# HTDerekLiu/surface_multigrid_code

Hardware: AMD Instinct MI355X
Metric: V-cycles/sec + fine-level SpMV GB/s (% HBM peak), 1M-vert mesh fp64 (higher is better)
Workload: dtype f64; 1 GPU; C3: bunny_15K_init x3 midpoint subdivision, 1011330 verts, 5 levels, M_bary+0.01(-L), fp64; n_verts=1011330, nnz=7079298, levels=5, smoother=gs, rhs_columns_per_gpu=1, parallelism=single GPU

## Files before the change

### surface_multigrid_code_amd/csrc/smg_capi.cpp

```cpp
#include <hip/hip_runtime.h>

#include <algorithm>
#include <atomic>
#include <chrono>
#include <cmath>
#include <cstdarg>
#include <cstdio>
#include <cstdlib>
#include <cstring>
#include <functional>
#include <memory>
#include <numeric>
#include <string>
#include <thread>
#include <vector>

#include "smg_internal.hpp"

using namespace smg;

static thread_local std::string g_err;
int smg::fail(int code, const char* fmt, ...)
{
    char buf[512];
    va_list ap;
    va_start(ap, fmt);
    std::vsnprintf(buf, sizeof(buf), fmt, ap);
    va_end(ap);
    g_err = buf;
    return code;
}

extern "C" const char* smg_last_error(void) { return g_err.c_str(); }
extern "C" int smg_version(void) { return SMG_VERSION; }
extern "C" long long smg_device_bytes_live(void) { return (long long)smg::devbuf_live_bytes().load(); }
extern "C" int smg_debug_device_bytes(const smg_hierarchy* h, char* buf, int cap)
{
    if (!h || !buf || cap < 1) return SMG_ERR_INVALID;
    std::string out;
    auto B = [](const auto& d) { return (long long)(d.n * sizeof(*d.p)); };
    auto sell = [&](const smg::SellBuf& S) { return B(S.slice_row) + B(S.slice_off) + B(S.slice_w) + B(S.col) + B(S.order) + B(S.val) + B(S.diag_slot) + B(S.long_row) + B(S.long_ptr) + B(S.long_col) + B(S.long_val) + B(S.long_valf); };
    long long tot = 0;
    auto line = [&](const std::string& nm, long long v) { if (v) { out += nm + " " + std::to_string(v) + "\n"; tot += v; } };
    for (int lv = 0; lv < h->n_levels; lv++) {
        const smg::Level& L = h->lv[lv];
        const std::string p = "level" + std::to_string(lv) + ".";
        line(p + "A_sell", sell(L.dA)); line(p + "AT_sell", sell(L.dAT)); line(p + "P_sell", sell(L.dP)); line(p + "PT_sell", sell(L.dPT));
        line(p + "A_block3", B(L.bA.slice_row) + B(L.bA.slice_off) + B(L.bA.slice_w) + B(L.bA.col) + B(L.bA.order) + B(L.bA.val) + B(L.bA.valf) + B(L.bAT.slice_row) + B(L.bAT.slice_off) + B(L.bAT.slice_w) + B(L.bAT.col) + B(L.bAT.order) + B(L.bAT.val) + B(L.bAT.valf) + B(L.mapB) + B(L.mapBT));
        line(p + "values_caller_order", B(L.d_Aval) + B(L.d_Tval));
        line(p + "refresh_maps", B(L.mapA) + B(L.mapAT));
        line(p + "galerkin_recipes", B(L.r1_ptr) + B(L.r1_idx) + B(L.r2_ptr) + B(L.r2_idx) + B(L.r1_coef) + B(L.r2_coef));
        long long t = 0;
        for (const auto& T : L.tiled) t += B(T.hdr) + B(T.ext_rows) + B(T.pcol) + B(T.prow) + B(T.map) + B(T.mapd) + B(T.pval) + B(T.pdiag);
        line(p + "tiled_plans", t);
        line(p + "bgs_plan", B(L.bgs.hdr) + B(L.bgs.xrow) + B(L.bgs.ugrow) + B(L.bgs.ulrow) + B(L.bgs.eidx) + B(L.bgs.map) + B(L.bgs.mapd) + B(L.bgs.eval) + B(L.bgs.udiag));
        line(p + "wgs_plan", B(L.wgs.hdr) + B(L.wgs.grow) + B(L.wgs.meta) + B(L.wgs.rim) + B(L.wgs.map) + B(L.wgs.mapd) + B(L.wgs.eoff) + B(L.wgs.eval) + B(L.wgs.diag));
        line(p + "fp32_images", B(L.a32) + B(L.at32) + B(L.p32) + B(L.pt32) + B(L.b32) + B(L.u32) + B(L.r32) + B(L.t32) + B(L.d32));
        line(p + "vectors", B(L.b) + B(L.u) + B(L.r) + B(L.t) + B(L.d));
    }
    line("coarse.dense_inverse", B(h->d_Ainv) + B(h->d_Ainv32));
    line("coarse.sym_partials", B(h->d_sympart));
    line("coarse.sparse_factor", B(h->c_perm) + B(h->c_rptr) + B(h->c_rcol) + B(h->c_cptr) + B(h->c_crow) + B(h->c_err) + B(h->c_rval) + B(h->c_cval) + B(h->c_diag) + B(h->c_work));
    line("coarse.schur", B(h->sch.irow) + B(h->sch.bsize) + B(h->sch.srow) + B(h->sch.sptr) + B(h->sch.sidx) + B(h->sch.aptr) + B(h->sch.ablk) + B(h->sch.acol) + B(h->sch.rptr) + B(h->sch.coff) + B(h->sch.pos) +
                         B(h->sch.pos2) + B(h->sch.ones) + B(h->sch.rdst) + B(h->sch.rdst2) + B(h->sch.rsrc) + B(h->sch.arena) + B(h->sch.g) + B(h->sch.xs) + B(h->sch.sym) + B(h->sch.gj) + B(h->sch.arena32) + B(h->sch.g32) + B(h->sch.xs32));
    line("maps_level0", B(h->d_map0) + B(h->d_perm0) + B(h->d_unknown) + B(h->d_known) + B(h->d_auk_ptr) + B(h->d_auk_col) + B(h->d_auk_val));
    line("reprecompute_bookkeeping", B(h->d_lhs_src) + B(h->d_auk_src) + B(h->d_diag_idx) + B(h->d_dense_pos) + B(h->d_Afull));
    line("early_upload", B(h->early0.ptr) + B(h->early0.col) + B(h->early0.val));
    line("solve_state", B(h->d_ctrl) + B(h->d_rhis) + B(h->d_partials) + B(h->d_lam) + B(h->d_stage_rhs) + B(h->d_stage_z) + B(h->d_stage_kv) + B(h->d_tmp_cm) + B(h->d_zsave));
    out += "total " + std::to_string(tot) + "\n";
    std::snprintf(buf, (size_t)cap, "%s", out.c_str());
    return SMG_OK;
}
extern "C" int smg_device_count(void)
{
    int n = 0;
    if (hipGetDeviceCount(&n) != hipSuccess) return 0;
    return n;
}
extern "C" void smg_solve_opts_default(smg_solve_opts* o)
{
    if (!o) return;
    o->tol = 1e-3;
    o->max_iter = 20;
    o->pre = 2;
    o->post = 2;
    o->verbosity = 0;
    o->check_every = 0;
    o->use_graph = 1;
    o->precision = 0;
    o->smoother = SMG_SMOOTH_GS;
    o->omega = 0.8;
    o->jacobi_max_rows = 100000;
    o->cheby_fraction = 0.1;
}

int smg::ensure_device(smg_hierarchy* h)
{
    if (h->device >= 0) return SMG_OK;
    int n = 0;
    if (hipGetDeviceCount(&n) != hipSuccess || n <= 0)
        return fail(SMG_ERR_NO_DEVICE, "no HIP device: libsmg has no CPU fallback (the CPU oracle lives in oracle/)");
    int dev = 0;
    HIPCHK(hipGetDevice(&dev));
    h->device = dev;
    if (!h->stream && !h->user_stream) {
        HIPCHK(hipStreamCreateWithFlags(&h->stream, hipStreamNonBlocking));
        h->own_stream = true;
    }
    HIPCHK(h->d_ctrl.alloc(1));
    HIPCHK(hipMemset(h->d_ctrl.p, 0, sizeof(Ctrl)));
    HIPCHK(h->d_rhis.alloc(1));
    return SMG_OK;
}

void smg::drop_graphs(smg_hierarchy* h)
{
    if (h->g_iter) (void)hipGraphExecDestroy(h->g_iter);
    if (h->g_iter_n) (void)hipGraphExecDestroy(h->g_iter_n);
    if (h->g_resid) (void)hipGraphExecDestroy(h->g_resid);
    if (h->g_cycle) (void)hipGraphExecDestroy(h->g_cycle);
    if (h->g_spec) (void)hipGraphExecDestroy(h->g_spec);
    if (h->g_rd) (void)hipGraphExecDestroy(h->g_rd);
    if (h->g_cyc) (void)hipGraphExecDestroy(h->g_cyc);
    h->g_iter = h->g_iter_n = h->g_resid = h->g_cycle = h->g_spec = h->g_rd = h->g_cyc = nullptr;
    h->g_key = smg::GraphKey();
}

hipError_t SellBuf::upload(const Sell& S)
{
    hipError_t e;
    if ((e = slice_row.upload(S.slice_row)) != hipSuccess) return e;
    if ((e = slice_off.upload(S.slice_off)) != hipSuccess) return e;
    if ((e = slice_w.upload(S.slice_w)) != hipSuccess) return e;
    const bool layout_only = S.col.empty() && S.padded() > 0;
    if (layout_only) {
        if ((e = col.alloc((size_t)S.padded())) != hipSuccess) return e;
        if ((e = val.alloc((size_t)S.padded())) != hipSuccess) return e;
    } else {
        if ((e = col.upload(S.col)) != hipSuccess) return e;
        if ((e = val.upload(S.val)) != hipSuccess) return e;
    }
    if ((e = order.upload(S.region_order)) != hipSuccess) return e;
    view.n_rows = S.n_rows; view.n_cols = S.n_cols; view.n_slices = S.n_slices; view.C = S.C;
    view.order = S.region_order.empty() ? nullptr : order.p;
    view.slice_row = slice_row.p; view.slice_off = slice_off.p; view.slice_w = slice_w.p; view.col = col.p; view.val = val.p;
    view.stride = S.stride; view.w_lo = S.w_lo;
    view.w_max = 0;
    for (int w : S.slice_w) view.w_max = std::max(view.w_max, w);
    if (env_int("SMG_DEBUG_SELL", 0)) {
        int hist[33] = {0};
        for (int w : S.slice_w) hist[std::min(w, 32)]++;
        std::fprintf(stderr, "sell %d x %d: %d slices, stride %d, w_lo %d, widths:", S.n_rows, S.n_cols, S.n_slices, S.stride, S.w_lo);
        for (int w = 0; w <= 32; w++) if (hist[w]) std::fprintf(stderr, " %d:%d", w, hist[w]);
        std::fprintf(stderr, "\n");
    }
    color_slice_ptr = S.color_slice_ptr;
    stored = S.nnz; padded = S.padded(); used = S.used();
    n_first = 0; n_all = 0;
    if (S.n_rows == S.n_cols && S.color_slice_ptr.size() >= 2 && !layout_only) {
        const int s1 = S.color_slice_ptr.size() >= 3 ? S.color_slice_ptr[1] : S.n_slices;
        const int nf = S.slice_row[s1];
        std::vector<int> slot((size_t)S.n_rows, -1);
        int first_missing = S.n_rows;
        for (int sl = 0; sl < S.n_slices; sl++) {
            const int r0 = S.slice_row[sl], r1 = S.slice_row[sl + 1];
            for (int r = r0; r < r1; r++) {
                for (int j = 0; j < S.slice_w[sl]; j++) {
                    const size_t at = ((size_t)S.slice_off[sl] + j) * S.C + (r - r0);
                    if (S.col[at] == r) { slot[r] = (int)at; break; }
                }
                if (slot[r] < 0 && r < first_missing) first_missing = r;
            }
        }
        if (S.n_rows > 0 && first_missing >= nf) {
            if ((e = diag_slot.upload(slot)) != hipSuccess) return e;
            if (S.color_slice_ptr.size() >= 3) n_first = nf;
            if (first_missing == S.n_rows) n_all = S.n_rows;
        }
    }
    return hipSuccess;
}

hipError_t SellBuf::upload_long(const std::vector<int>& rows, const std::vector<int>& ptr, const std::vector<int>& col, const std::vector<double>& val)
{
    hipError_t e;
    view.long_n = 0; view.long_row = view.long_ptr = view.long_col = nullptr; view.long_val = nullptr; view.long_valf = nullptr;
    long_valf.release();
    if (rows.empty()) { long_row.release(); long_ptr.release(); long_col.release(); long_val.release(); return hipSuccess; }
    if ((e = long_row.upload(rows)) != hipSuccess) return e;
    if ((e = long_ptr.upload(ptr)) != hipSuccess) return e;
    if ((e = long_col.upload(col)) != hipSuccess) return e;
    if ((e = long_val.upload(val)) != hipSuccess) return e;
    view.long_n = (int)rows.size(); view.long_row = long_row.p; view.long_ptr = long_ptr.p; view.long_col = long_col.p; view.long_val = long_val.p;
    return hipSuccess;
}

hipError_t Bsr3Buf::upload(const Bsr3Sell& S)
{
    hipError_t e;
    if ((e = slice_row.upload(S.slice_row)) != hipSuccess) return e;
    if ((e = slice_off.upload(S.slice_off)) != hipSuccess) return e;
    if ((e = slice_w.upload(S.slice_w)) != hipSuccess) return e;
    const size_t slots = (size_t)64 * (size_t)(S.slice_off.empty() ? 0 : S.slice_off.back());
    const bool layout_only = S.col.empty() && slots > 0;
    if (layout_only) {
        if ((e = col.alloc(slots)) != hipSuccess) return e;
        if ((e = val.alloc(slots * 9)) != hipSuccess) return e;
    } else {
        if ((e = col.upload(S.col)) != hipSuccess) return e;
        if ((e = val.upload(S.val)) != hipSuccess) return e;
    }
    if ((e = order.upload(S.region_order)) != hipSuccess) return e;
    view.n_vert = S.n_vert; view.n_slices = S.n_slices; view.w_max = S.w_max;
    view.slice_row = slice_row.p; view.slice_off = slice_off.p; view.slice_w = slice_w.p; view.col = col.p; view.val = val.p;
    view.order = S.region_order.empty() ? nullptr : order.p;
    color_slice_ptr = S.color_slice_ptr;
    stored = S.nnz_scalar; blocks = S.n_blocks; padded = (long)(slots * 9);
    return hipSuccess;
}

int smg::prof_scope_id(smg_hierarchy* h, const char* name)
{
    for (size_t i = 0; i < h->scopes.size(); i++) if (h->scopes[i].name == name) return (int)i;
    ProfScope s; s.name = name;
    h->scopes.push_back(s);
    return (int)h->scopes.size() - 1;
}
hipEvent_t smg::prof_event(smg_hierarchy* h)
{
    if (!h->ev_pool.empty()) { hipEvent_t e = h->ev_pool.back(); h->ev_pool.pop_back(); return e; }
    hipEvent_t e = nullptr;
    (void)hipEventCreate(&e);
    return e;
}
void smg::prof_collect(smg_hierarchy* h)
{
    if (h->recs.empty()) return;
    (void)hipStreamSynchronize(h->stream);
    for (auto& r : h->recs) {
        float ms = 0.f;
        if (hipEventElapsedTime(&ms, r.e0, r.e1) == hipSuccess) { h->scopes[r.scope].ms += ms; h->scopes[r.scope].count++; }
        h->ev_pool.push_back(r.e0); h->ev_pool.push_back(r.e1);
    }
    h->recs.clear();
}

extern "C" smg_hierarchy* smg_hierarchy_create(int n_levels)
{
    if (n_levels < 1) { fail(SMG_ERR_INVALID, "n_levels must be >= 1"); return nullptr; }
    smg_hierarchy* h = new (std::nothrow) smg_hierarchy();
    if (!h) { fail(SMG_ERR_ALLOC, "out of memory"); return nullptr; }
    h->n_levels = n_levels;
    h->lv.resize(n_levels);
    h->coarse_dense_max = env_int("SMG_COARSE_DENSE_MAX", 16384);
    h->coarse_dense_max_user = std::getenv("SMG_COARSE_DENSE_MAX") != nullptr;
    h->bgs_min_rows = env_int("SMG_BGS_MIN_ROWS", -1);
    h->coarse_schur_when = std::min(2, std::max(0, env_int("SMG_COARSE_SCHUR", 2)));
    h->coarse_schur_min = env_int("SMG_COARSE_SCHUR_MIN", 2048);
    h->coarse_schur_big = env_int("SMG_COARSE_SCHUR_BIG", 6144);
    h->coarse_schur_max = env_int("SMG_COARSE_SCHUR_MAX", 65536);
    return h;
}

extern "C" void smg_hierarchy_destroy(smg_hierarchy* h)
{
    if (!h) return;
    if (h->stream) (void)hipStreamSynchronize(h->stream);
    drop_graphs(h);
    for (auto& r : h->recs) { (void)hipEventDestroy(r.e0); (void)hipEventDestroy(r.e1); }
    for (auto e : h->ev_pool) (void)hipEventDestroy(e);
    if (h->own_stream && h->stream) (void)hipStreamDestroy(h->stream);
    for (hipStream_t a : h->aux) if (a) (void)hipStreamDestroy(a);
    delete h;
}

extern "C" int smg_hierarchy_levels(const smg_hierarchy* h) { return h ? h->n_levels : SMG_ERR_INVALID; }

extern "C" int smg_hierarchy_set_stream(smg_hierarchy* h, void* hip_stream)
{
    if (!h) return fail(SMG_ERR_INVALID, "null handle");
    if (h->stream) (void)hipStreamSynchronize(h->stream);
    drop_graphs(h);
    if (h->own_stream && h->stream) (void)hipStreamDestroy(h->stream);
    h->stream = (hipStream_t)hip_stream;
    h->own_stream = false;
    h->user_stream = true;
    return SMG_OK;
}

extern "C" int smg_hierarchy_set_smoother(smg_hierarchy* h, int smoother, double omega, int jacobi_max_rows)
{
    if (!h) return fail(SMG_ERR_INVALID, "null handle");
    if (smoother < SMG_SMOOTH_GS || smoother > SMG_SMOOTH_HYBRID_CHEBYSHEV)
        return fail(SMG_ERR_INVALID, "smoother must be one of SMG_SMOOTH_GS, _JACOBI, _HYBRID, _CHEBYSHEV, _HYBRID_CHEBYSHEV");
    if (h->in_solve) return fail(SMG_ERR_INVALID, "smg_hierarchy_set_smoother called during a split-phase solve");
    if (omega > 2.0 || omega != omega) return fail(SMG_ERR_INVALID, "omega must be in (0, 2]");
    h->smoother = smoother;
    if (omega > 0.0) h->omega = omega;
    if (jacobi_max_rows >= 0) h->jacobi_max_rows = jacobi_max_rows;
    return SMG_OK;
}

extern "C" int smg_hierarchy_set_block_mode(smg_hierarchy* h, int mode)
{
    if (!h) return fail(SMG_ERR_INVALID, "null handle");
    if (mode != -1 && mode != 0 && mode != 3) return fail(SMG_ERR_INVALID, "smg_hierarchy_set_block_mode: mode must be -1 (automatic), 0 (scalar) or 3");
    if (h->in_solve) return fail(SMG_ERR_INVALID, "smg_hierarchy_set_block_mode called during a split-phase solve");
    if (mode != h->block_mode) { h->block_mode = mode; h->precomputed = false; }
    return SMG_OK;
}
extern "C" int smg_hierarchy_block_size(const smg_hierarchy* h) { return h ? h->bs : SMG_ERR_INVALID; }
extern "C" int smg_level_block_stats(const smg_hierarchy* h, int lv, long* n_blocks, long* n_block_slots, int* n_vertex_colors)
{
    if (!h || lv < 0 || lv >= h->n_levels - 1) return fail(SMG_ERR_INVALID, "smg_level_block_stats: bad level");
    if (h->bs != 3 || !h->precomputed) return fail(SMG_ERR_INVALID, "smg_level_block_stats: not a precomputed block hierarchy");
    const Bsr3Buf& B = h->lv[lv].bA;
    if (n_blocks) *n_blocks = B.blocks;
    if (n_block_slots) *n_block_slots = B.padded / 9;
    if (n_vertex_colors) *n_vertex_colors = h->lv[lv].vord.n_colors();
    return SMG_OK;
}

extern "C" int smg_level_get_block_image(const smg_hierarchy* h, int lv, int* n_slices, int* n_panel_cols, int* slice_row, int* slice_off, int* slice_w,
                                         int* col, double* val)
{
    return guarded("smg_level_get_block_image", [&]() {
        if (!h || lv < 0 || lv >= h->n_levels - 1) return fail(SMG_ERR_INVALID, "smg_level_get_block_image: bad level");
        const Level& Lv = h->lv[lv];
        if (h->bs != 3 || Lv.A_int.nr != Lv.n || Lv.n == 0 || (int)Lv.vord.perm.size() * 3 != Lv.n)
            return fail(SMG_ERR_INVALID, "smg_level_get_block_image: the host half of smg_precompute has not run on a block hierarchy");
        const Bsr3Sell S = build_bsr3(Lv.A_int, &Lv.vord.color_ptr, false);
        if (n_slices) *n_slices = S.n_slices;
        if (n_panel_cols) *n_panel_cols = S.slice_off.back();
        if (slice_row) std::copy(S.slice_row.begin(), S.slice_row.end(), slice_row);
        if (slice_off) std::copy(S.slice_off.begin(), S.slice_off.end(), slice_off);
        if (slice_w) std::copy(S.slice_w.begin(), S.slice_w.end(), slice_w);
        if (col) std::copy(S.col.begin(), S.col.end(), col);
        if (val) std::copy(S.val.begin(), S.val.end(), val);
        return (int)SMG_OK;
    });
}

extern "C" int smg_hierarchy_set_coarse_dense_max(smg_hierarchy* h, int n_max)
{
    if (!h || n_max < 0) return fail(SMG_ERR_INVALID, "smg_hierarchy_set_coarse_dense_max: bad arguments");
    if (h->in_solve) return fail(SMG_ERR_INVALID, "smg_hierarchy_set_coarse_dense_max called during a split-phase solve");
// ... 683 lines not shown
```

### surface_multigrid_code_amd/csrc/smg_cycle.cpp

```cpp
#include <hip/hip_runtime.h>

#include <algorithm>
#include <chrono>
#include <cmath>
#include <cstdarg>
#include <cstdio>
#include <cstdlib>
#include <cstring>
#include <functional>
#include <memory>
#include <numeric>
#include <string>
#include <thread>
#include <vector>

#include "smg_internal.hpp"

using namespace smg;


static hipError_t ensure_map(DevBuf<int>& d, const std::vector<int>& host)
{
    if (d.n == host.size() && (d.p || host.empty())) return hipSuccess;
    return d.upload(host);
// ... 171 lines not shown
    if (Lv.n < min_rows || Lv.n > max_rows) return false;
    if (mode == 1) return true;
    const SellBuf& Gs = Lv.gs_on_transpose ? Lv.dAT : Lv.dA;
    return Lv.ord.n_colors() > TILED_NCMAX || Gs.view.w_max > TILED_WMAX;
}
static const WgsBuf* wgs_plan(const smg_hierarchy* h, int lv, int k)
{
    if (!wgs_wanted(h, lv, k)) return nullptr;
    const WgsBuf& B = h->lv[lv].wgs;
    return B.view.n_pieces > 0 ? &B : nullptr;
}
static int ensure_wgs(smg_hierarchy* h, int lv)
{
    Level& Lv = h->lv[lv];
    WgsBuf& B = Lv.wgs;
    if (B.tried) return SMG_OK;
    B.tried = true;
    static const int rows_env = env_int("SMG_WGS_ROWS", WGS_ROWS), mode_env = env_int("SMG_WGS_PIECES", 1);
    std::vector<int> tsrc;
    Csr AT;
    { int rc = ensure_A_int(h, lv); if (rc) return rc; }
    if (Lv.gs_on_transpose) AT = transpose(Lv.A_int, &tsrc);
    const Csr& G = Lv.gs_on_transpose ? AT : Lv.A_int;
    const auto t_plan0 = std::chrono::steady_clock::now();
    WgsPlan P = build_wgs(G, std::min(std::max(rows_env, 8), (int)WGS_ROWS), mode_env);
    const double plan_ms = 1e3 * std::chrono::duration<double>(std::chrono::steady_clock::now() - t_plan0).count();
    if (P.empty()) return SMG_OK;
    auto to_level_value = [&](const std::vector<int>& entries) {
        std::vector<int> m(entries.size());
        for (size_t i = 0; i < m.size(); i++) {
            const int e = entries[i];
            m[i] = e < 0 ? -1 : Lv.A_int_src[(size_t)(Lv.gs_on_transpose ? tsrc[(size_t)e] : e)];
        }
        return m;
    };
    const std::vector<int> map = to_level_value(P.eentry), mapd = to_level_value(P.dentry);
    HIPCHK(B.hdr.upload(P.hdr)); HIPCHK(B.grow.upload(P.grow)); HIPCHK(B.meta.upload(P.meta)); HIPCHK(B.diag.upload(P.diag)); HIPCHK(B.rim.upload(P.rim));
    HIPCHK(B.eoff.upload(P.eoff)); HIPCHK(B.eval.upload(P.eval)); B.host_map = map; B.host_mapd = mapd;
    B.view.n_pieces = P.n_pieces; B.view.n_colors = P.n_colors; B.view.rim_pitch = P.rim_pitch; B.view.nb_max = P.nb_max;
    B.view.hdr = B.hdr.p; B.view.grow = B.grow.p; B.view.meta = B.meta.p; B.view.diag = B.diag.p; B.view.rim = B.rim.p; B.view.eoff = B.eoff.p; B.view.eval = B.eval.p;
    B.color_ptr = P.color_ptr; B.host_rows = P.rows; B.host_piece_ptr = P.piece_ptr; B.rim_ratio = P.rim_ratio; B.phases_mean = P.phases_mean; B.phases_max = P.phases_max;
    if (h->host_stale && Lv.d_Aval.p) {
        HIPCHK(ensure_map(B.map, B.host_map)); HIPCHK(ensure_map(B.mapd, B.host_mapd));
        HIPCHK(launch_gather_vals(B.eval.p, Lv.d_Aval.p, B.map.p, B.eval.n, h->stream));
        HIPCHK(launch_gather_vals(B.diag.p, Lv.d_Aval.p, B.mapd.p, B.diag.n, h->stream));
    }
    if (env_int("SMG_DEBUG_WGS", 0))
        std::fprintf(stderr, "wave Gauss-Seidel level %d: %d rows, %d pieces in %d colours, phases per piece %.1f (max %d), rim %.2f rows read per row beyond the iterate, rim pitch %d; plan built in %.0f ms\n",
                     lv, Lv.n, P.n_pieces, P.n_colors, P.phases_mean, P.phases_max, P.rim_ratio, P.rim_pitch, plan_ms);
    return SMG_OK;
}

int smg::prepare_level_plans(smg_hierarchy* h, int lv)
{
    static const int on = env_int("SMG_EARLY_PLANS", 1), max_rows = env_int("SMG_EARLY_PLANS_MAX_ROWS", 70000);
    if (!on || lv <= 0 || lv >= h->n_levels - 1 || h->precision != 0 || h->lv[lv].n > max_rows) return SMG_OK;
    const int sa = h->pre, sb = h->post;
    for (int sw : {sa, sb}) if (sw > 0 && tiled_wanted(h, lv, 1, sw)) { int rc = ensure_tiled(h, lv, sw); if (rc) return rc; }
    if (wgs_wanted(h, lv, 1) && !h->lv[lv].wgs.tried && !tiled_plan(h, lv, 1, sa) && !tiled_plan(h, lv, 1, sb)) { int rc = ensure_wgs(h, lv); if (rc) return rc; }
    return SMG_OK;
}

static int prepare_tiled(smg_hierarchy* h, int k, int sa, int sb)
{
    for (int lv = 0; lv < h->n_levels - 1; lv++) {
        Level& Lv = h->lv[lv];
        for (int sw : {sa, sb}) if (tiled_wanted(h, lv, k, sw)) { int rc = ensure_tiled(h, lv, sw); if (rc) return rc; }
        if (bgs_wanted(h, lv, k) && !Lv.bgs.tried) { drop_graphs(h); int rc = ensure_bgs(h, lv); if (rc) return rc; }
        if (wgs_wanted(h, lv, k) && !Lv.wgs.tried && !tiled_plan(h, lv, k, sa) && !tiled_plan(h, lv, k, sb)) { drop_graphs(h); int rc = ensure_wgs(h, lv); if (rc) return rc; }
        if ((tiled_plan(h, lv, k, sa) || tiled_plan(h, lv, k, sb)) && Lv.t.n < (size_t)Lv.n * std::max(h->kcap, 1)) {
            drop_graphs(h);
            HIPCHK(Lv.t.alloc((size_t)Lv.n * std::max(h->kcap, 1)));
            HIPCHK(hipMemsetAsync(Lv.t.p, 0, Lv.t.n * sizeof(double), h->stream));
        }
    }
    return SMG_OK;
}

static int ensure_work(smg_hierarchy* h, int k)
{
    const int L = h->n_levels;
    if (k > h->kcap) {
        drop_graphs(h);
        size_t maxblocks = 0;
        for (int lv = 0; lv < L; lv++) {
            Level& Lv = h->lv[lv];
            size_t rows = (lv == L - 1) ? (size_t)h->nc_pad : (size_t)Lv.n;
            HIPCHK(Lv.b.alloc(rows * k));
            HIPCHK(Lv.u.alloc(rows * k));
            HIPCHK(hipMemsetAsync(Lv.b.p, 0, rows * k * sizeof(double), h->stream));
            HIPCHK(hipMemsetAsync(Lv.u.p, 0, rows * k * sizeof(double), h->stream));
            Lv.t.release(); Lv.d.release();
            if (lv < L - 1 || L == 1) HIPCHK(Lv.r.alloc(rows * k));
            if (lv < L - 1 || L == 1) {
                if (h->bs == 3) maxblocks = std::max(maxblocks, (size_t)bsr3_blocks(Lv.bA.view.n_slices) * (size_t)k);
                else maxblocks = std::max(maxblocks, (size_t)sell_blocks(Lv.dA.view.n_slices) * ((k + 3) / 4) + (size_t)sell_wide_blocks(Lv.dA.view.n_slices, k));
            }
        }
        maxblocks += (h->lv[0].dA.color_slice_ptr.size() + 1) * (size_t)((k + 3) / 4 + 8);
        HIPCHK(h->d_partials.alloc(std::max<size_t>(maxblocks, 1) + (size_t)ss_partials_room()));
        h->kcap = k;
    }
    for (int lv = 0; lv < L - 1; lv++) {
        Level& Lv = h->lv[lv];
        if ((level_is_jacobi(h, lv) || lv == 0) && Lv.t.n < (size_t)Lv.n * h->kcap) {
            drop_graphs(h);
            HIPCHK(Lv.t.alloc((size_t)Lv.n * h->kcap));
            HIPCHK(hipMemsetAsync(Lv.t.p, 0, (size_t)Lv.n * h->kcap * sizeof(double), h->stream));
        }
        if (level_kind(h, lv) == LV_CHEBY && Lv.d.n < (size_t)Lv.n * h->kcap) {
            drop_graphs(h);
            HIPCHK(Lv.d.alloc((size_t)Lv.n * h->kcap));
            HIPCHK(hipMemsetAsync(Lv.d.p, 0, (size_t)Lv.n * h->kcap * sizeof(double), h->stream));
        }
    }
    if (h->coarse_schur) {
        const size_t need = (size_t)h->sch.view.ns_pad * std::max(h->kcap, 1);
        if (h->sch.g.n < need || h->sch.xs.n < need) {
            drop_graphs(h);
            HIPCHK(h->sch.g.alloc(need));
            HIPCHK(h->sch.xs.alloc(need));
            HIPCHK(hipMemsetAsync(h->sch.g.p, 0, need * sizeof(double), h->stream));
            HIPCHK(hipMemsetAsync(h->sch.xs.p, 0, need * sizeof(double), h->stream));
        }
        h->sch.view.g = h->sch.g.p; h->sch.view.xs = h->sch.xs.p;
    }
    if (h->coarse_sparse) {
        const size_t need = (size_t)2 * h->chol.n * sparse_coarse_work_cols(std::max(h->kcap, 1));
        if (h->c_work.n < need) {
            drop_graphs(h);
            HIPCHK(h->c_work.alloc(need));
            h->c_view.work = h->c_work.p;
        }
    }
    int rc = prepare_tiled(h, k, h->pre, h->post);
    if (rc) return rc;
    return ensure_spectral_bounds(h);
}

static int ensure_fp32(smg_hierarchy* h, int k)
{
    const int L = h->n_levels;
    if (h->union_m > 0) return fail(SMG_ERR_INVALID, "a union handle solves in fp64 (its coarse inverses are per-member blocks: no fp32 image)");
    if (h->coarse_sparse) return fail(SMG_ERR_INVALID, "the mixed-precision cycle is not available with a sparse coarse factorisation (coarsest level of %d unknowns)", h->nc);
    if (!h->f32_valid) {
        drop_graphs(h);
        auto mk = [&](SellBuf& src, DevBuf<float>& dst, SellDev& view) -> int {
            if (src.view.long_n > 0) {
                HIPCHK(src.long_valf.ensure(src.long_val.n));
                HIPCHK(launch_cvt_f64_f32(src.long_valf.p, src.long_val.p, src.long_val.n, h->stream));
                src.view.long_valf = src.long_valf.p;
            }
            view = src.view;
            if (src.padded == 0) { view.valf = nullptr; return SMG_OK; }
            HIPCHK(dst.ensure((size_t)src.padded));
            HIPCHK(launch_cvt_f64_f32(dst.p, src.view.val, (size_t)src.padded, h->stream));
            view.valf = dst.p;
            return SMG_OK;
        };
        for (int lv = 0; lv < L; lv++) {
            Level& Lv = h->lv[lv];
            int rc;
            if (lv < L - 1 && h->bs == 3) {
                auto mkb = [&](Bsr3Buf& B) -> int {
                    HIPCHK(B.valf.ensure(B.val.n));
                    HIPCHK(launch_cvt_f64_f32(B.valf.p, B.val.p, B.val.n, h->stream));
                    B.view.valf = B.valf.p;
                    return SMG_OK;
                };
                if ((rc = mkb(Lv.bA))) return rc;
                if (Lv.gs_on_transpose) { if ((rc = mkb(Lv.bAT))) return rc; }
            } else if (lv < L - 1) {
                if ((rc = mk(Lv.dA, Lv.a32, Lv.dA32))) return rc;
                if (Lv.gs_on_transpose) { if ((rc = mk(Lv.dAT, Lv.at32, Lv.dAT32))) return rc; }
            }
            if (lv >= 1) {
                if ((rc = mk(Lv.dP, Lv.p32, Lv.dP32))) return rc;
                if ((rc = mk(Lv.dPT, Lv.pt32, Lv.dPT32))) return rc;
            }
        }
        if (h->coarse_schur) {
            HIPCHK(h->sch.arena32.ensure((size_t)h->schur.off_C));
            HIPCHK(launch_cvt_f64_f32(h->sch.arena32.p, h->sch.arena.p, (size_t)h->schur.off_C, h->stream));
            h->sch.view.arena32 = h->sch.arena32.p;
        } else {
            HIPCHK(h->d_Ainv32.ensure((size_t)h->nc_pad * h->nc_pad));
            HIPCHK(launch_cvt_f64_f32(h->d_Ainv32.p, h->d_Ainv.p, (size_t)h->nc_pad * h->nc_pad, h->stream));
        }
        h->f32_valid = true;
    }
    if (k > h->kcap32) {
        drop_graphs(h);
        for (int lv = 0; lv < L; lv++) {
            Level& Lv = h->lv[lv];
            const size_t rows = (lv == L - 1) ? (size_t)h->nc_pad : (size_t)Lv.n;
            HIPCHK(Lv.b32.alloc(rows * k));
            HIPCHK(Lv.u32.alloc(rows * k));
            HIPCHK(hipMemsetAsync(Lv.b32.p, 0, rows * k * sizeof(float), h->stream));
            HIPCHK(hipMemsetAsync(Lv.u32.p, 0, rows * k * sizeof(float), h->stream));
            if (lv < L - 1) HIPCHK(Lv.r32.alloc(rows * k));
            Lv.t32.release(); Lv.d32.release();
        }
        h->kcap32 = k;
    }
    for (int lv = 0; lv < L - 1; lv++) {
        Level& Lv = h->lv[lv];
        if (level_is_jacobi(h, lv) && Lv.t32.n < (size_t)Lv.n * h->kcap32) {
            drop_graphs(h);
            HIPCHK(Lv.t32.alloc((size_t)Lv.n * h->kcap32));
            HIPCHK(hipMemsetAsync(Lv.t32.p, 0, (size_t)Lv.n * h->kcap32 * sizeof(float), h->stream));
        }
        if (level_kind(h, lv) == LV_CHEBY && Lv.d32.n < (size_t)Lv.n * h->kcap32) {
            drop_graphs(h);
            HIPCHK(Lv.d32.alloc((size_t)Lv.n * h->kcap32));
            HIPCHK(hipMemsetAsync(Lv.d32.p, 0, (size_t)Lv.n * h->kcap32 * sizeof(float), h->stream));
        }
    }
    if (h->coarse_schur) {
        const size_t need = (size_t)h->sch.view.ns_pad * std::max(h->kcap32, 1);
        if (h->sch.g32.n < need || h->sch.xs32.n < need) {
            drop_graphs(h);
            HIPCHK(h->sch.g32.alloc(need));
            HIPCHK(h->sch.xs32.alloc(need));
            HIPCHK(hipMemsetAsync(h->sch.g32.p, 0, need * sizeof(float), h->stream));
            HIPCHK(hipMemsetAsync(h->sch.xs32.p, 0, need * sizeof(float), h->stream));
        }
        h->sch.view.g32 = h->sch.g32.p; h->sch.view.xs32 = h->sch.xs32.p;
    }
    return SMG_OK;
}

int smg::level_kind(const smg_hierarchy* h, int lv)
{
    if (lv < 0 || lv >= h->n_levels - 1) return LV_GS;
    switch (h->smoother) {
        case SMG_SMOOTH_JACOBI: return LV_JACOBI;
        case SMG_SMOOTH_HYBRID: return h->lv[lv].n <= h->jacobi_max_rows ? LV_JACOBI : LV_GS;
        case SMG_SMOOTH_CHEBYSHEV: return LV_CHEBY;
        case SMG_SMOOTH_HYBRID_CHEBYSHEV: return h->lv[lv].n <= h->jacobi_max_rows ? LV_CHEBY : LV_GS;
    }
    return LV_GS;
}

struct ChebyCoef { double c1, c2; };
static void cheby_coefs(double lam, double frac, int degree, std::vector<ChebyCoef>& out)
{
    out.resize((size_t)std::max(degree, 0));
    const double lmax = lam, lmin = lam * frac;
    const double theta = (lmax + lmin) / 2.0, delta = (lmax - lmin) / 2.0;
    const double sigma = theta / delta;
    double rho = 1.0 / sigma;
    for (int s = 0; s < degree; s++) {
        if (s == 0) { out[s].c1 = 0.0; out[s].c2 = 1.0 / theta; }
        else {
            const double rho_new = 1.0 / (2.0 * sigma - rho);
            out[s].c1 = rho_new * rho;
            out[s].c2 = 2.0 * rho_new / delta;
            rho = rho_new;
        }
    }
}

template <typename T> struct Prec;
static inline int coarse_cols(const smg_hierarchy* h, int k) { return (h->coarse_cols > 0 && h->coarse_cols < k) ? h->coarse_cols : k; }

template <> struct Prec<double> {
    static double* b(Level& L) { return L.b.p; }
    static double* u(Level& L) { return L.u.p; }
    static double* r(Level& L) { return L.r.p; }
    static double* t(Level& L) { return L.t.p; }
    static double* d(Level& L) { return L.d.p; }
    static void set_d(FirstColour& fc, Level& L) { fc.d = L.d.p; }
    static const SellDev& A(Level& L) { return L.dA.view; }
    static const SellDev& G(Level& L) { return L.gs_on_transpose ? L.dAT.view : L.dA.view; }
    static const SellDev& P(Level& L) { return L.dP.view; }
    static const SellDev& PT(Level& L) { return L.dPT.view; }
    static bool has_vals(const SellDev& V) { return V.val != nullptr; }
    static hipError_t sell(SellMode m, const SellDev& V, int s0, int s1, const double* x, const double* bb, double* y, int k, const Ctrl* ctrl,
                           hipStream_t st, double* zero_rows = nullptr, const FirstColour* first = nullptr, double omega = 1.0)
    { return launch_sell(m, V, s0, s1, x, bb, y, k, ctrl, nullptr, nullptr, st, zero_rows, first, omega); }
    static hipError_t coarse(smg_hierarchy* h, Level& L, int k, const Ctrl* ctrl)
    {
        if (h->union_m > 0) return launch_blockdiag_gemv_add(h->un.view, h->d_Ainv.p, h->nc, L.b.p, L.u.p, k, ctrl, h->stream);
        if (h->coarse_sparse) return launch_sparse_coarse_solve(h->c_view, L.b.p, L.u.p, k, ctrl, h->stream);
        if (h->coarse_schur) return launch_schur_solve(h->sch.view, L.b.p, L.u.p, k, ctrl, h->stream);
        return launch_dense_gemv_add(h->d_Ainv.p, h->nc, h->nc_pad, L.b.p, L.u.p, coarse_cols(h, k), k, ctrl, h->stream, h->d_sympart.p);
    }
    static hipError_t opA(smg_hierarchy* h, Level& L, bool smoother_image, SellMode m, int s0, int s1, const double* x, const double* bb, double* y, int k,
                          const Ctrl* ctrl, const FirstColour* fc = nullptr, double omega = 1.0)
    {
        if (h->bs == 3) {
            const Bsr3Dev& V = (smoother_image && L.gs_on_transpose) ? L.bAT.view : L.bA.view;
            return launch_bsr3(m, V, s0, s1 < 0 ? V.n_slices : s1, x, bb, y, k, ctrl, nullptr, nullptr, h->stream, omega, fc ? fc->c1 : 0.0, fc ? fc->d : nullptr);
        }
        const SellDev& V = smoother_image ? G(L) : A(L);
        return sell(m, V, s0, s1 < 0 ? V.n_slices : s1, x, bb, y, k, ctrl, h->stream, nullptr, fc, omega);
    }
};
template <> struct Prec<float> {
    static float* b(Level& L) { return L.b32.p; }
    static float* u(Level& L) { return L.u32.p; }
    static float* r(Level& L) { return L.r32.p; }
    static float* t(Level& L) { return L.t32.p; }
    static float* d(Level& L) { return L.d32.p; }
    static void set_d(FirstColour& fc, Level& L) { fc.df = L.d32.p; }
    static const SellDev& A(Level& L) { return L.dA32; }
    static const SellDev& G(Level& L) { return L.gs_on_transpose ? L.dAT32 : L.dA32; }
// ... 1127 lines not shown
```

### surface_multigrid_code_amd/csrc/smg_device.hip

```cpp
#include <hip/hip_runtime.h>

#include <cstdlib>
#include <type_traits>

#include "smg_device.hpp"
#include "smg_device_inl.hpp"
#include "smg_gj_inl.hpp"

namespace smg {


__device__ int g_never_done = 0;
const int* never_done()
{
    static const int* p = nullptr;
    if (!p) { void* q = nullptr; if (hipGetSymbolAddress(&q, HIP_SYMBOL(g_never_done)) == hipSuccess) p = (const int*)q; }
    return p;
}


template <typename T> struct CoarseInit { T* u; const T* gs_val; const int* diag_slot; int n_first; int jacobi; T omega; T* d; T c1; };

template <int MODE, int KB, typename T, int W0C = -1, int WPB = 4>
__global__ __launch_bounds__(64 * WPB) void k_sell(const int* a_col, const T* a_val, const int* a_order, const int* a_slice_off, int a_stride,
                                              int a_w_lo, int s_begin, int s_end, int n_blocks, int use_order, const T* x,
                                              const int* a_slice_row, const int* a_slice_w, const T* b, T* y, int ld, const int* done,
                                              double* partials, CoarseInit<T> z)
{
    struct { const int *slice_row, *slice_off, *slice_w, *order, *col; int stride, w_lo; } A = {a_slice_row, a_slice_off, a_slice_w, a_order,
                                                                                               a_col, a_stride, a_w_lo};
    constexpr int C = 64;
    const int lane = threadIdx.x & 63;
    const int wave = threadIdx.x >> 6;
    constexpr int wpb = WPB;
    constexpr bool GS = sell_is_gs(MODE), OOP = sell_is_oop(MODE), JAC = sell_is_jacobi(MODE), CHEB = sell_is_cheby(MODE), HEAD = sell_is_head(MODE);
    int bid;
    if (GS && n_blocks < 0) { if (blockIdx.x & 7) return; bid = blockIdx.x >> 3; }
    else bid = xcd_remap(blockIdx.x, n_blocks);
    const int ls = __builtin_amdgcn_readfirstlane(s_begin + bid * wpb + wave);
    double ss = 0.0;
    int stop = 0;
    if (ls < s_end) {
        const int s = (!GS && use_order) ? A.order[ls] : ls;
        const int W0 = W0C >= 0 ? W0C : (A.w_lo < 8 ? A.w_lo : 8);
        const int off0 = (W0C >= 0 || A.stride) ? s * A.stride : A.slice_off[s];
        const int* cp = A.col + (size_t)off0 * C + lane;
        const T* vp = a_val + (size_t)off0 * C + lane;
        constexpr int U = W0C > 8 ? W0C : 8;
        int c0[U];
        T v0[U];
#pragma unroll
        for (int t = 0; t < U; t++) {
            if (t < W0) { c0[t] = cp[(size_t)t * C]; v0[t] = vp[(size_t)t * C]; }
            else { c0[t] = -1; v0[t] = (T)0; }
        }
        {
            size_t keep = (size_t)x ^ (size_t)A.slice_row ^ (size_t)A.slice_w ^ (size_t)b ^ (size_t)y ^ (size_t)done ^ (size_t)ld;
            if (MODE == SELL_AX) keep ^= (size_t)z.u ^ (size_t)z.gs_val ^ (size_t)z.diag_slot ^ (size_t)z.n_first ^ (size_t)z.jacobi ^ (size_t)z.d;
            if (CHEB) keep ^= (size_t)z.d;
            asm("" : "+s"(keep));
            if (keep == 0x5a5a5a5a5a5a5a5bull) return;
        }
        stop = load_flag(done);
        const int row0 = A.slice_row[s];
        const int nrow = A.slice_row[s + 1] - row0;
        const int w = A.slice_w[s];
        const int rowb = row0 + lane;
        const int split = OOP ? A.slice_row[s_begin] : 0;
        T acc[KB];
        T accr[KB];
        T diag = (T)1;
        T xi[KB];
        T dold[KB];
        T bv[KB];
        const bool live = lane < nrow;
        T zd = (T)1;
        if (MODE == SELL_AX && live && rowb < z.n_first) zd = z.gs_val[z.diag_slot[rowb]];
#pragma unroll
        for (int q = 0; q < KB; q++) {
            acc[q] = (T)0; accr[q] = (T)0; xi[q] = (T)0; dold[q] = (T)0;
            if (MODE == SELL_AX) bv[q] = (T)0;
            else bv[q] = live ? b[(size_t)rowb * ld + q] : (T)0;
            if (CHEB && live && z.c1 != (T)0) dold[q] = z.d[(size_t)rowb * ld + q];
        }
        auto consume = [&](const int (&c)[U], const T (&v)[U]) {
            T xv[U][KB];
            T xo[MODE == SELL_GS_HEAD ? U : 1][KB];
#pragma unroll
            for (int t = 0; t < U; t++) {
                const bool use = (c[t] >= 0) && !(GS && c[t] == rowb);
                if constexpr (MODE == SELL_GS_HEAD) {
                    gather_kb<KB, T>(x + (size_t)c[t] * ld, c[t] >= 0, xo[t]);
                    gather_kb<KB, T>((const T*)y + (size_t)c[t] * ld, use && c[t] < split, xv[t]);
                } else if constexpr (MODE == SELL_GS_OOP) {
                    gather_kb<KB, T>((c[t] < split ? (const T*)y : x) + (size_t)c[t] * ld, use, xv[t]);
                } else {
                    gather_kb<KB, T>(x + (size_t)c[t] * ld, use, xv[t]);
                }
            }
#pragma unroll
            for (int t = 0; t < U; t++) {
                if (c[t] >= 0) {
                    if (HEAD) {
#pragma unroll
                        for (int q = 0; q < KB; q++) accr[q] += v[t] * (MODE == SELL_GS_HEAD ? xo[t][q] : xv[t][q]);
                    }
                    if (GS && c[t] == rowb) {
                        diag = v[t];
                    } else if ((JAC || CHEB) && c[t] == rowb) {
                        diag = v[t];
#pragma unroll
                        for (int q = 0; q < KB; q++) xi[q] = xv[t][q];
                    } else {
#pragma unroll
                        for (int q = 0; q < KB; q++) acc[q] += v[t] * ((MODE == SELL_GS_HEAD && c[t] >= split) ? xo[t][q] : xv[t][q]);
                    }
                }
            }
        };
        if (W0 > 0) consume(c0, v0);
        for (int j0 = W0; j0 < w; j0 += U) {
            int c[U];
            T v[U];
#pragma unroll
            for (int t = 0; t < U; t++) {
                if ((j0 + t) < w) { c[t] = cp[(size_t)(j0 + t) * C]; v[t] = vp[(size_t)(j0 + t) * C]; }
                else { c[t] = -1; v[t] = (T)0; }
            }
            consume(c, v);
        }
        if (live && !stop) {
            const size_t o = (size_t)rowb * ld;
#pragma unroll
            for (int q = 0; q < KB; q++) {
                if (MODE == SELL_AX) {
                    y[o + q] = acc[q];
                    if (z.u) {
                        const T t = acc[q] / zd;
                        if (z.jacobi == 2) { const T dn = z.omega * (t - (T)0); z.u[o + q] = (T)0 + dn; z.d[o + q] = dn; }
                        else z.u[o + q] = rowb < z.n_first ? (z.jacobi ? (T)0 + z.omega * (t - (T)0) : t) : (T)0;
                    }
                }
                else if (MODE == SELL_RESID) y[o + q] = bv[q] - acc[q];
                else if (MODE == SELL_ADD) y[o + q] = bv[q] + acc[q];
                else if (GS) y[o + q] = (bv[q] - acc[q]) / diag;
                else if (JAC) { const T t = (bv[q] - acc[q]) / diag; y[o + q] = xi[q] + z.omega * (t - xi[q]); }
                else if (CHEB) {
                    const T t = (bv[q] - acc[q]) / diag;
                    const T r = t - xi[q];
                    const T dn = z.c1 != (T)0 ? z.c1 * dold[q] + z.omega * r : z.omega * r;
                    y[o + q] = xi[q] + dn;
                    z.d[o + q] = dn;
                }
                else { const double t = (double)(bv[q] - acc[q]); ss += t * t; if (MODE == SELL_RESID_BOTH) y[o + q] = bv[q] - acc[q]; }
                if (HEAD) { const double t = (double)(bv[q] - accr[q]); ss += t * t; }
            }
        }
    }
    if (sell_has_ss(MODE)) {
        __shared__ double red[16];
#pragma unroll
        for (int o = 32; o > 0; o >>= 1) ss += __shfl_down(ss, o, 64);
        if (lane == 0) red[wave] = ss;
        __syncthreads();
        if (threadIdx.x == 0 && !stop) {
            double t = 0.0;
            for (int i2 = 0; i2 < wpb; i2++) t += red[i2];
            partials[HEAD ? bid : (int)blockIdx.x] = t;
        }
    }
}

template <int MODE, int KB, int NBMAX>
__global__ __launch_bounds__(256) void k_sell_deep(const int* a_col, const double* a_val, const int* a_order, const int* a_slice_off, int a_stride, int s_begin, int s_end,
                                                   int n_blocks, int use_order, const double* x, const int* a_slice_row, const int* a_slice_w, const double* b, double* y, int ld,
                                                   const int* done, CoarseInit<double> z)
{
    constexpr int C = 64, S = NBMAX * 8;
    const int lane = threadIdx.x & 63, wave = threadIdx.x >> 6;
    const int bid = xcd_remap(blockIdx.x, n_blocks);
    const int ls = __builtin_amdgcn_readfirstlane(s_begin + bid * 4 + wave);
    if (ls >= s_end) return;
    const int s = use_order ? a_order[ls] : ls;
    const int stop = load_flag(done);
    const int oz = __builtin_amdgcn_mbcnt_lo(~0u, 0u) >> 6;
    const int row0 = a_slice_row[s + oz], nrow = a_slice_row[s + 1 + oz] - row0, w = a_slice_w[s + oz];
    const int off0 = a_stride ? s * a_stride : a_slice_off[s + oz];
    const int rowb = row0 + lane;
    const bool live = lane < nrow;
    const int* cp = a_col + (size_t)off0 * C + lane;
    const double* vp = a_val + (size_t)off0 * C + lane;
    int c[S];
    double v[S];
#pragma unroll
    for (int bt = 0; bt < NBMAX; bt++) {
        if (bt * 8 < w) {
#pragma unroll
            for (int t = bt * 8; t < bt * 8 + 8; t++) {
                const int tt = t < w ? t : w - 1;
                c[t] = cp[(size_t)tt * C];
                v[t] = vp[(size_t)tt * C];
            }
        } else {
#pragma unroll
            for (int t = bt * 8; t < bt * 8 + 8; t++) { c[t] = -1; v[t] = 0.0; }
        }
    }
    double zd = 1.0, bv[KB];
    if (MODE == SELL_AX && live && rowb < z.n_first) zd = z.gs_val[z.diag_slot[rowb]];
#pragma unroll
    for (int q = 0; q < KB; q++) bv[q] = (MODE == SELL_RESID && live) ? b[(size_t)rowb * ld + q] : 0.0;
    double xv[S][KB];
#pragma unroll
    for (int t = 0; t < S; t++) {
        const bool use = c[t] >= 0 && t < w;
        if (!use) v[t] = 0.0;
        gather_kb<KB, double>(x + (size_t)(use ? c[t] : 0) * ld, use, xv[t]);
    }
    double acc[KB];
#pragma unroll
    for (int q = 0; q < KB; q++) acc[q] = 0.0;
#pragma unroll
    for (int bt = 0; bt < NBMAX; bt++) {
        if (bt * 8 < w) {
#pragma unroll
            for (int t = bt * 8; t < bt * 8 + 8; t++)
#pragma unroll
                for (int q = 0; q < KB; q++) acc[q] += v[t] * xv[t][q];
        }
    }
    if (live && !stop) {
        const size_t o = (size_t)rowb * ld;
#pragma unroll
        for (int q = 0; q < KB; q++) {
            if (MODE == SELL_AX) {
                y[o + q] = acc[q];
                if (z.u) {
                    const double t = acc[q] / zd;
                    if (z.jacobi == 2) { const double dn = z.omega * (t - 0.0); z.u[o + q] = 0.0 + dn; z.d[o + q] = dn; }
                    else z.u[o + q] = rowb < z.n_first ? (z.jacobi ? 0.0 + z.omega * (t - 0.0) : t) : 0.0;
                }
            } else y[o + q] = bv[q] - acc[q];
        }
    }
}
static bool deep_wanted(int mode, int w_max, int kb)
{
    static const int on = getenv("SMG_DEEP") ? atoi(getenv("SMG_DEEP")) : 1;
    static const int wmin = getenv("SMG_DEEP_MIN_W") ? atoi(getenv("SMG_DEEP_MIN_W")) : 13;
    if (!on || (mode != SELL_AX && mode != SELL_RESID) || w_max < wmin || w_max > 64) return false;
    const int nbm = w_max <= 24 ? 3 : w_max <= 40 ? 5 : 8;
    return nbm == 3 ? kb <= 3 : nbm == 5 ? kb <= 2 : kb == 1;
}

template <int MODE, int KW, typename T, int R = 2, int U = 8>
__global__ __launch_bounds__(256) void k_sell_wide(const int* a_col, const T* a_val, const int* a_order, const int* a_slice_off, int a_stride,
                                                   int s_begin, int s_end, int n_blocks, int use_order, const T* x,
                                                   const int* a_slice_row, const int* a_slice_w, const T* b, T* y, int ld,
                                                   const int* done, double* partials, CoarseInit<T> z)
{
    struct { const int *slice_row, *slice_off, *slice_w, *order, *col; int stride; } A = {a_slice_row, a_slice_off, a_slice_w, a_order, a_col,
                                                                                        a_stride};
    constexpr bool GS = sell_is_gs(MODE), OOP = sell_is_oop(MODE), JAC = sell_is_jacobi(MODE), CHEB = sell_is_cheby(MODE), HEAD = sell_is_head(MODE);
    const int stop = load_flag(done);
    constexpr int G = 64 / KW;
    constexpr int RW = R * G;
    constexpr int SUB = 64 / RW;
    const int lane = threadIdx.x & 63;
    const int wave = threadIdx.x >> 6;
    const int c = lane % KW, g = lane / KW;
    const int bid = xcd_remap(blockIdx.x, n_blocks);
    const int wid = __builtin_amdgcn_readfirstlane(bid * 4 + wave);
    const int ls = s_begin + wid / SUB;
    const int sub = wid % SUB;
    double ss = 0.0;
    if (ls < s_end) {
        const int s = use_order ? A.order[ls] : ls;
        const int row0 = A.slice_row[s];
        const int nrow = A.slice_row[s + 1] - row0;
        const int off0 = A.stride ? s * A.stride : A.slice_off[s];
        const int w = A.slice_w[s];
        const int split = OOP ? A.slice_row[s_begin] : 0;
        int rl[R];
        T acc[R], accr[R], diag[R], bv[R], zd[R], xi[R], dold[R];
#pragma unroll
        for (int r = 0; r < R; r++) {
            rl[r] = sub * RW + r * G + g;
            acc[r] = (T)0; accr[r] = (T)0; diag[r] = (T)1; xi[r] = (T)0; dold[r] = (T)0;
            const bool live = rl[r] < nrow;
            zd[r] = (T)1;
            if (MODE == SELL_AX && live && row0 + rl[r] < z.n_first) zd[r] = z.gs_val[z.diag_slot[row0 + rl[r]]];
            const size_t o = (size_t)(row0 + rl[r]) * ld + c;
            if (MODE == SELL_AX) bv[r] = (T)0;
            else bv[r] = live ? b[o] : (T)0;
            if (CHEB && live && z.c1 != (T)0) dold[r] = z.d[o];
        }
        const int* cp = A.col + (size_t)off0 * 64;
        const T* vp = a_val + (size_t)off0 * 64;
        for (int j0 = 0; j0 < w; j0 += U) {
            int cc[U][R];
            T vv[U][R], xv[U][R];
            T xo[MODE == SELL_GS_HEAD ? U : 1][R];
            constexpr int NL = G == 1 ? 1 : (U * RW + 63) / 64;
            int cL[NL];
            T vL[NL];
            if constexpr (G > 1) {
#pragma unroll
                for (int q = 0; q < NL; q++) {
                    const int e = q * 64 + lane, tt = e / RW, rr = e % RW;
                    const bool in2 = e < U * RW && (j0 + tt) < w;
                    cL[q] = in2 ? cp[(size_t)(j0 + tt) * 64 + sub * RW + rr] : -1;
                    vL[q] = in2 ? vp[(size_t)(j0 + tt) * 64 + sub * RW + rr] : (T)0;
                }
            }
#pragma unroll
            for (int t = 0; t < U; t++)
#pragma unroll
                for (int r = 0; r < R; r++) {
                    const bool in = (j0 + t) < w;
                    (void)in;
                    if constexpr (G == 1) {
                        cc[t][r] = in ? cp[(size_t)(j0 + t) * 64 + rl[r]] : -1;
                        vv[t][r] = in ? vp[(size_t)(j0 + t) * 64 + rl[r]] : (T)0;
                    } else {
                        const int src = t * RW + r * G + g;
                        cc[t][r] = __shfl(cL[(t * RW + r * G) / 64], src & 63, 64);
                        vv[t][r] = __shfl(vL[(t * RW + r * G) / 64], src & 63, 64);
                    }
                }
#pragma unroll
            for (int t = 0; t < U; t++)
#pragma unroll
                for (int r = 0; r < R; r++) {
                    const bool use = (cc[t][r] >= 0) && !(GS && cc[t][r] == row0 + rl[r]);
                    if constexpr (MODE == SELL_GS_HEAD) {
                        xo[t][r] = cc[t][r] >= 0 ? x[(size_t)cc[t][r] * ld + c] : (T)0;
                        xv[t][r] = (use && cc[t][r] < split) ? y[(size_t)cc[t][r] * ld + c] : (T)0;
                    } else if constexpr (MODE == SELL_GS_OOP) {
                        const T* src = cc[t][r] < split ? (const T*)y : x;
                        xv[t][r] = use ? src[(size_t)cc[t][r] * ld + c] : (T)0;
                    } else xv[t][r] = use ? x[(size_t)cc[t][r] * ld + c] : (T)0;
                }
#pragma unroll
            for (int t = 0; t < U; t++)
#pragma unroll
                for (int r = 0; r < R; r++) {
                    if (cc[t][r] >= 0) {
                        if (HEAD) accr[r] += vv[t][r] * (MODE == SELL_GS_HEAD ? xo[t][r] : xv[t][r]);
                        if (GS && cc[t][r] == row0 + rl[r]) diag[r] = vv[t][r];
                        else if ((JAC || CHEB) && cc[t][r] == row0 + rl[r]) { diag[r] = vv[t][r]; xi[r] = xv[t][r]; }
                        else acc[r] += vv[t][r] * ((MODE == SELL_GS_HEAD && cc[t][r] >= split) ? xo[t][r] : xv[t][r]);
                    }
                }
        }
#pragma unroll
        for (int r = 0; r < R; r++) {
            if (rl[r] < nrow && !stop) {
                const size_t o = (size_t)(row0 + rl[r]) * ld + c;
                if (MODE == SELL_AX) {
                    y[o] = acc[r];
                    if (z.u) {
                        const T t = acc[r] / zd[r];
                        if (z.jacobi == 2) { const T dn = z.omega * (t - (T)0); z.u[o] = (T)0 + dn; z.d[o] = dn; }
                        else z.u[o] = row0 + rl[r] < z.n_first ? (z.jacobi ? (T)0 + z.omega * (t - (T)0) : t) : (T)0;
                    }
                }
                else if (MODE == SELL_RESID) y[o] = bv[r] - acc[r];
                else if (MODE == SELL_ADD) y[o] = bv[r] + acc[r];
                else if (GS) y[o] = (bv[r] - acc[r]) / diag[r];
                else if (JAC) { const T t = (bv[r] - acc[r]) / diag[r]; y[o] = xi[r] + z.omega * (t - xi[r]); }
                else if (CHEB) {
                    const T t = (bv[r] - acc[r]) / diag[r];
                    const T rr = t - xi[r];
                    const T dn = z.c1 != (T)0 ? z.c1 * dold[r] + z.omega * rr : z.omega * rr;
                    y[o] = xi[r] + dn;
                    z.d[o] = dn;
                }
                else { const double t = (double)(bv[r] - acc[r]); ss += t * t; if (MODE == SELL_RESID_BOTH) y[o] = bv[r] - acc[r]; }
                if (HEAD) { const double t = (double)(bv[r] - accr[r]); ss += t * t; }
            }
        }
    }
    if (sell_has_ss(MODE)) {
        __shared__ double red[4];
#pragma unroll
        for (int o = 32; o > 0; o >>= 1) ss += __shfl_down(ss, o, 64);
        if (lane == 0) red[wave] = ss;
        __syncthreads();
        if (threadIdx.x == 0 && !stop) partials[blockIdx.x] = (red[0] + red[1]) + (red[2] + red[3]);
    }
}

template <typename T>
__global__ __launch_bounds__(256) void k_long_ax(const int* rows, const int* ptr, const int* col, const T* val, int nl, const T* x, T* y, int ld, int k,
                                                 const int* done, CoarseInit<T> z)
{
    const int stop = load_flag(done);
    const int lane = threadIdx.x & 63;
    const long wid = (long)blockIdx.x * 4 + (threadIdx.x >> 6);
    if (wid >= (long)nl * k) return;
    const int r = (int)(wid / k), c = (int)(wid % k);
    const int row = rows[r], p0 = ptr[r], p1 = ptr[r + 1];
    T zd = (T)1;
    if (z.u && row < z.n_first) zd = z.gs_val[z.diag_slot[row]];
    T acc = (T)0;
    for (int base = p0; base < p1; base += 64) {
        const int t = base + lane;
        T prod = (T)0;
        if (t < p1) prod = val[t] * x[(size_t)col[t] * ld + c];
        const int n = (p1 - base) < 64 ? (p1 - base) : 64;
        for (int i = 0; i < n; i++) acc += __shfl(prod, i, 64);
    }
    if (lane == 0 && !stop) {
        const size_t o = (size_t)row * ld + c;
        y[o] = acc;
        if (z.u) {
            const T t = acc / zd;
            if (z.jacobi == 2) { const T dn = z.omega * (t - (T)0); z.u[o] = (T)0 + dn; z.d[o] = dn; }
            else z.u[o] = row < z.n_first ? (z.jacobi ? (T)0 + z.omega * (t - (T)0) : t) : (T)0;
        }
    }
}
template <typename T>
__global__ __launch_bounds__(256) void k_long_ax_cols(const int* rows, const int* ptr, const int* col, const T* val, int nl, const T* x, T* y, int ld, int k,
                                                      const int* done, CoarseInit<T> z)
{
    const int stop = load_flag(done);
    const int lane = threadIdx.x & 63;
    const int cblocks = (k + 63) >> 6;
    const long wid = (long)blockIdx.x * 4 + (threadIdx.x >> 6);
    if (wid >= (long)nl * cblocks) return;
    const int r = (int)(wid / cblocks), c = (int)(wid % cblocks) * 64 + lane;
    const bool colok = c < k;
    const int row = rows[r], p0 = ptr[r], p1 = ptr[r + 1];
    T zd = (T)1;
    if (z.u && row < z.n_first) zd = z.gs_val[z.diag_slot[row]];
    T acc = (T)0;
    constexpr int U = 32;
    for (int base = p0; base < p1; base += 64) {
        const int t = base + lane;
        const int ce = t < p1 ? col[t] : 0;
        const T ve = t < p1 ? val[t] : (T)0;
        const int n = (p1 - base) < 64 ? (p1 - base) : 64;
        for (int i0 = 0; i0 < n; i0 += U) {
            T xv[U], vv[U];
#pragma unroll
            for (int i = 0; i < U; i++) {
                const int cc = __shfl(ce, (i0 + i) & 63, 64);
                vv[i] = __shfl(ve, (i0 + i) & 63, 64);
                xv[i] = (i0 + i < n && colok) ? x[(size_t)cc * ld + c] : (T)0;
            }
#pragma unroll
            for (int i = 0; i < U; i++) if (i0 + i < n) acc += vv[i] * xv[i];
        }
    }
    if (colok && !stop) {
        const size_t o = (size_t)row * ld + c;
        y[o] = acc;
        if (z.u) {
            const T t = acc / zd;
            if (z.jacobi == 2) { const T dn = z.omega * (t - (T)0); z.u[o] = (T)0 + dn; z.d[o] = dn; }
            else z.u[o] = row < z.n_first ? (z.jacobi ? (T)0 + z.omega * (t - (T)0) : t) : (T)0;
        }
    }
}
template <typename T> static const T* host_long_vals(const SellDev& A);
template <> const double* host_long_vals<double>(const SellDev& A) { return A.long_val; }
template <> const float* host_long_vals<float>(const SellDev& A) { return A.long_valf; }

template <typename T> static const T* host_vals(const SellDev& A);
template <typename T> static CoarseInit<T> coarse_init(T* zero_rows, int c0, const FirstColour* first, double omega)
{
    CoarseInit<T> z{zero_rows ? zero_rows + c0 : nullptr, nullptr, nullptr, 0, 0, (T)omega, nullptr, (T)0};
    if (first) {
        if constexpr (std::is_same<T, double>::value) z.d = first->d ? first->d + c0 : nullptr; else z.d = first->df ? first->df + c0 : nullptr;
        z.c1 = (T)first->c1;
    }
    if (zero_rows && first && first->n_first > 0) {
        if constexpr (std::is_same<T, double>::value) z.gs_val = first->val; else z.gs_val = first->valf;
        z.diag_slot = first->diag_slot;
        z.n_first = (z.gs_val && z.diag_slot) ? first->n_first : 0;
        z.jacobi = first->jacobi;
        if (first->jacobi) z.omega = (T)first->omega;
    }
    return z;
}
template <> const double* host_vals<double>(const SellDev& A) { return A.val; }
template <> const float* host_vals<float>(const SellDev& A) { return A.valf; }

static long wide_latency_max()
{
    static const long v = getenv("SMG_WIDE_LAT_MAX") ? atol(getenv("SMG_WIDE_LAT_MAX")) : 16384;
    return v;
}
static bool wide_latency_variant(int n_slices, int kw) { return (long)n_slices * kw <= wide_latency_max(); }

template <int MODE, int KW, typename T>
static void launch_wide_one(const SellDev& A, int s_begin, int s_end, int use_order, const T* x, const T* b, T* y,
                            int k, const int* done, double* partials, CoarseInit<T> zero_rows, hipStream_t st, int* nb_out)
{
    const int ns = s_end - s_begin;
    if constexpr (KW < 64) if (wide_latency_variant(ns, KW)) {
        const int nb = (ns * KW + 3) / 4;
#define SMG_WIDE_LAT(UU) hipLaunchKernelGGL((k_sell_wide<MODE, KW, T, 1, UU>), dim3(nb), dim3(256), 0, st, A.col, host_vals<T>(A), A.order, A.slice_off, A.stride, \
                                             s_begin, s_end, nb, use_order, x, A.slice_row, A.slice_w, b, y, k, done, partials, zero_rows)
        if (A.w_max <= 8) SMG_WIDE_LAT(8);
        else if (A.w_max <= 16) SMG_WIDE_LAT(16);
        else SMG_WIDE_LAT(32);
#undef SMG_WIDE_LAT
        *nb_out = nb;
        return;
    }
    const int waves = ns * (KW / 2);
    const int nb = (waves + 3) / 4;
    hipLaunchKernelGGL((k_sell_wide<MODE, KW, T>), dim3(nb), dim3(256), 0, st, A.col, host_vals<T>(A), A.order, A.slice_off, A.stride, s_begin, s_end, nb, use_order, x,
                       A.slice_row, A.slice_w, b, y, k, done, partials, zero_rows);
    *nb_out = nb;
}

int sell_wide_blocks(int n_slices, int k)
{
    int tot = 0, c0 = 0;
    while (k - c0 >= 8) { int kw = 64; while (kw > k - c0) kw >>= 1; tot += (n_slices * kw + 3) / 4; c0 += kw; }
    return tot;
}

static constexpr int sell_wpb() { return 4; }
static int gs_wpb() { static const int v = getenv("SMG_GS_WPB") ? atoi(getenv("SMG_GS_WPB")) : 4; return v; }
int sell_blocks(int n_slices) { return (n_slices + sell_wpb() - 1) / sell_wpb(); }

template <int MODE, typename T>
static hipError_t launch_sell_mode(const SellDev& A, int s_begin, int s_end_in, const T* x, const T* b, T* y,
                                   int k, const Ctrl* ctrl, double* partials, int* n_blocks, hipStream_t st, T* zero_rows, const FirstColour* first,
                                   double omega)
{
    int s_end = s_end_in;
    if (MODE == SELL_ADD && !b) b = y;
    const int ns = s_end - s_begin;
    const int nb = sell_blocks(ns);
    const int* done = ctrl ? &ctrl->done : never_done();
    static const int dbg_empty = getenv("SMG_DEBUG_EMPTY") ? atoi(getenv("SMG_DEBUG_EMPTY")) : 0;
    if (dbg_empty == 1) s_end = s_begin;
    const int use_order = (A.order && s_begin == 0 && s_end == A.n_slices) ? 1 : 0;
    if (n_blocks) *n_blocks = 0;
    if (ns <= 0) return hipSuccess;
    int c0 = 0;
    size_t poff = 0;
    {
        while (k - c0 >= 8) {
            int kw = 64;
            while (kw > k - c0) kw >>= 1;
            const T* xx = x ? x + c0 : nullptr;
            const T* bb = b ? b + c0 : nullptr;
            T* yy = y ? y + c0 : nullptr;
            double* pp = partials ? partials + poff : nullptr;
            const CoarseInit<T> zz = coarse_init<T>(zero_rows, c0, first, omega);
            int wnb = 0;
            switch (kw) {
                case 64: launch_wide_one<MODE, 64, T>(A, s_begin, s_end, use_order, xx, bb, yy, k, done, pp, zz, st, &wnb); break;
                case 32: launch_wide_one<MODE, 32, T>(A, s_begin, s_end, use_order, xx, bb, yy, k, done, pp, zz, st, &wnb); break;
                case 16: launch_wide_one<MODE, 16, T>(A, s_begin, s_end, use_order, xx, bb, yy, k, done, pp, zz, st, &wnb); break;
                default: launch_wide_one<MODE, 8, T>(A, s_begin, s_end, use_order, xx, bb, yy, k, done, pp, zz, st, &wnb); break;
            }
            poff += (size_t)wnb;
            c0 += kw;
        }
    }
    static const int one_xcd_max = getenv("SMG_ONE_XCD_MAX") ? atoi(getenv("SMG_ONE_XCD_MAX")) : 32;
    const bool one_xcd = sell_is_gs(MODE) && nb <= one_xcd_max;
    const int grid = one_xcd ? nb * 8 : nb, nbarg = one_xcd ? -nb : nb;
    for (; c0 < k; c0 += 4) {
        const int kb = (k - c0) < 4 ? (k - c0) : 4;
        const T* xx = x ? x + c0 : nullptr;
        const T* bb = b ? b + c0 : nullptr;
        T* yy = y ? y + c0 : nullptr;
        double* pp = partials ? partials + poff : nullptr;
        const CoarseInit<T> zz = coarse_init<T>(zero_rows, c0, first, omega);
        poff += (size_t)nb;
        if constexpr (std::is_same<T, double>::value && (MODE == SELL_AX || MODE == SELL_RESID)) {
            int kd = kb;
            if (kd == 4 && !deep_wanted(MODE, A.w_max, 4) && deep_wanted(MODE, A.w_max, 2)) kd = 2;
            if (deep_wanted(MODE, A.w_max, kd) || (kd > 1 && deep_wanted(MODE, A.w_max, 1))) {
                for (int cc = 0; cc < kb;) {
                    int kk = kb - cc;
                    while (kk > 1 && !deep_wanted(MODE, A.w_max, kk)) kk--;
                    const int nbm = A.w_max <= 24 ? 3 : A.w_max <= 40 ? 5 : 8;
                    const CoarseInit<T> zc = coarse_init<T>(zero_rows, c0 + cc, first, omega);
#define SMG_DEEP_LAUNCH(KB, NB) hipLaunchKernelGGL((k_sell_deep<MODE, KB, NB>), dim3(nb), dim3(256), 0, st, A.col, A.val, A.order, A.slice_off, A.stride, s_begin, s_end, nb, use_order, \
                                                   xx ? xx + cc : nullptr, A.slice_row, A.slice_w, bb ? bb + cc : nullptr, yy + cc, k, done, zc)
                    if (nbm == 3) { if (kk == 1) SMG_DEEP_LAUNCH(1, 3); else if (kk == 2) SMG_DEEP_LAUNCH(2, 3); else SMG_DEEP_LAUNCH(3, 3); }
                    else if (nbm == 5) { if (kk == 1) SMG_DEEP_LAUNCH(1, 5); else SMG_DEEP_LAUNCH(2, 5); }
                    else SMG_DEEP_LAUNCH(1, 8);
#undef SMG_DEEP_LAUNCH
                    cc += kk;
                }
                continue;
            }
        }
        switch (kb) {
            case 1: {
                const int w0 = A.stride > 0 ? (A.w_lo < 8 ? A.w_lo : 8) : -1;
                static const int pitch_env = getenv("SMG_PITCH_SPEC_MAX") ? atoi(getenv("SMG_PITCH_SPEC_MAX")) : -1;
                const int pitch_max = pitch_env >= 0 ? pitch_env : (sell_is_gs(MODE) ? 32 : 64);
                if (nb <= pitch_max && A.stride == 12 && w0 >= 7) hipLaunchKernelGGL((k_sell<MODE, 1, T, 12>), dim3(grid), dim3(64 * sell_wpb()), 0, st, A.col, host_vals<T>(A), A.order, A.slice_off, A.stride, A.w_lo, s_begin, s_end, nbarg, use_order, xx, A.slice_row, A.slice_w, bb, yy, k, done, pp, zz);
                else if (w0 == 7 && MODE == SELL_GS && !one_xcd && gs_wpb() == 8) hipLaunchKernelGGL((k_sell<MODE == SELL_GS ? MODE : SELL_GS, 1, T, 7, 8>), dim3((ns + 7) / 8), dim3(512), 0, st, A.col, host_vals<T>(A), A.order, A.slice_off, A.stride, A.w_lo, s_begin, s_end, (ns + 7) / 8, use_order, xx, A.slice_row, A.slice_w, bb, yy, k, done, pp, zz);
                else if (w0 == 7 && MODE == SELL_GS && !one_xcd && gs_wpb() == 2) hipLaunchKernelGGL((k_sell<MODE == SELL_GS ? MODE : SELL_GS, 1, T, 7, 2>), dim3((ns + 1) / 2), dim3(128), 0, st, A.col, host_vals<T>(A), A.order, A.slice_off, A.stride, A.w_lo, s_begin, s_end, (ns + 1) / 2, use_order, xx, A.slice_row, A.slice_w, bb, yy, k, done, pp, zz);
                else if (w0 == 7) hipLaunchKernelGGL((k_sell<MODE, 1, T, 7>), dim3(grid), dim3(64 * sell_wpb()), 0, st, A.col, host_vals<T>(A), A.order, A.slice_off, A.stride, A.w_lo, s_begin, s_end, nbarg, use_order, xx, A.slice_row, A.slice_w, bb, yy, k, done, pp, zz);
                else if (w0 == 8) hipLaunchKernelGGL((k_sell<MODE, 1, T, 8>), dim3(grid), dim3(64 * sell_wpb()), 0, st, A.col, host_vals<T>(A), A.order, A.slice_off, A.stride, A.w_lo, s_begin, s_end, nbarg, use_order, xx, A.slice_row, A.slice_w, bb, yy, k, done, pp, zz);
                else if (w0 == 2) hipLaunchKernelGGL((k_sell<MODE, 1, T, 2>), dim3(grid), dim3(64 * sell_wpb()), 0, st, A.col, host_vals<T>(A), A.order, A.slice_off, A.stride, A.w_lo, s_begin, s_end, nbarg, use_order, xx, A.slice_row, A.slice_w, bb, yy, k, done, pp, zz);
                else hipLaunchKernelGGL((k_sell<MODE, 1, T>), dim3(grid), dim3(64 * sell_wpb()), 0, st, A.col, host_vals<T>(A), A.order, A.slice_off, A.stride, A.w_lo, s_begin, s_end, nbarg, use_order, xx, A.slice_row, A.slice_w, bb, yy, k, done, pp, zz);
                break;
            }
            case 2:
                if (A.stride > 0 && A.w_lo == 7) hipLaunchKernelGGL((k_sell<MODE, 2, T, 7>), dim3(grid), dim3(64 * sell_wpb()), 0, st, A.col, host_vals<T>(A), A.order, A.slice_off, A.stride, A.w_lo, s_begin, s_end, nbarg, use_order, xx, A.slice_row, A.slice_w, bb, yy, k, done, pp, zz);
                else hipLaunchKernelGGL((k_sell<MODE, 2, T>), dim3(grid), dim3(64 * sell_wpb()), 0, st, A.col, host_vals<T>(A), A.order, A.slice_off, A.stride, A.w_lo, s_begin, s_end, nbarg, use_order, xx, A.slice_row, A.slice_w, bb, yy, k, done, pp, zz);
                break;
            case 3:
                if (A.stride > 0 && A.w_lo == 7) hipLaunchKernelGGL((k_sell<MODE, 3, T, 7>), dim3(grid), dim3(64 * sell_wpb()), 0, st, A.col, host_vals<T>(A), A.order, A.slice_off, A.stride, A.w_lo, s_begin, s_end, nbarg, use_order, xx, A.slice_row, A.slice_w, bb, yy, k, done, pp, zz);
                else hipLaunchKernelGGL((k_sell<MODE, 3, T>), dim3(grid), dim3(64 * sell_wpb()), 0, st, A.col, host_vals<T>(A), A.order, A.slice_off, A.stride, A.w_lo, s_begin, s_end, nbarg, use_order, xx, A.slice_row, A.slice_w, bb, yy, k, done, pp, zz);
                break;
            default:
                if (A.stride > 0 && A.w_lo == 7) hipLaunchKernelGGL((k_sell<MODE, 4, T, 7>), dim3(grid), dim3(64 * sell_wpb()), 0, st, A.col, host_vals<T>(A), A.order, A.slice_off, A.stride, A.w_lo, s_begin, s_end, nbarg, use_order, xx, A.slice_row, A.slice_w, bb, yy, k, done, pp, zz);
                else hipLaunchKernelGGL((k_sell<MODE, 4, T>), dim3(grid), dim3(64 * sell_wpb()), 0, st, A.col, host_vals<T>(A), A.order, A.slice_off, A.stride, A.w_lo, s_begin, s_end, nbarg, use_order, xx, A.slice_row, A.slice_w, bb, yy, k, done, pp, zz);
                break;
        }
    }
    if (MODE == SELL_AX && A.long_n > 0 && s_begin == 0 && s_end_in == A.n_slices && host_long_vals<T>(A)) {
        const CoarseInit<T> zz = coarse_init<T>(zero_rows, 0, first, omega);
        if (k >= 8) {
            const long waves = (long)A.long_n * ((k + 63) / 64);
            hipLaunchKernelGGL((k_long_ax_cols<T>), dim3((unsigned)((waves + 3) / 4)), dim3(256), 0, st, A.long_row, A.long_ptr, A.long_col, host_long_vals<T>(A), A.long_n, x, y,
                               k, k, done, zz);
        } else {
            const long waves = (long)A.long_n * k;
            hipLaunchKernelGGL((k_long_ax<T>), dim3((unsigned)((waves + 3) / 4)), dim3(256), 0, st, A.long_row, A.long_ptr, A.long_col, host_long_vals<T>(A), A.long_n, x, y, k, k,
                               done, zz);
        }
    }
    if (n_blocks) *n_blocks = (int)poff;
    return hipGetLastError();
}

template <typename T>
static hipError_t launch_sell_any(SellMode mode, const SellDev& A, int s_begin, int s_end, const T* x, const T* b,
                                  T* y, int k, const Ctrl* ctrl, double* partials, int* n_blocks, hipStream_t st,
                                  T* zero_rows, const FirstColour* first, double omega)
{
    switch (mode) {
        case SELL_JACOBI: return launch_sell_mode<SELL_JACOBI, T>(A, s_begin, s_end, x, b, y, k, ctrl, partials, n_blocks, st, zero_rows, first, omega);
        case SELL_CHEBY: return launch_sell_mode<SELL_CHEBY, T>(A, s_begin, s_end, x, b, y, k, ctrl, partials, n_blocks, st, zero_rows, first, omega);
        case SELL_AX: return launch_sell_mode<SELL_AX, T>(A, s_begin, s_end, x, b, y, k, ctrl, partials, n_blocks, st, zero_rows, first, omega);
        case SELL_RESID: return launch_sell_mode<SELL_RESID, T>(A, s_begin, s_end, x, b, y, k, ctrl, partials, n_blocks, st, zero_rows, first, omega);
        case SELL_RESID_SS:
            if constexpr (std::is_same<T, double>::value) return launch_sell_mode<SELL_RESID_SS, T>(A, s_begin, s_end, x, b, y, k, ctrl, partials, n_blocks, st, zero_rows, first, omega);
            else return hipErrorInvalidValue;
        case SELL_ADD: return launch_sell_mode<SELL_ADD, T>(A, s_begin, s_end, x, b, y, k, ctrl, partials, n_blocks, st, zero_rows, first, omega);
        case SELL_GS: return launch_sell_mode<SELL_GS, T>(A, s_begin, s_end, x, b, y, k, ctrl, partials, n_blocks, st, zero_rows, first, omega);
        case SELL_RESID_BOTH:
            if constexpr (std::is_same<T, double>::value) return launch_sell_mode<SELL_RESID_BOTH, T>(A, s_begin, s_end, x, b, y, k, ctrl, partials, n_blocks, st, zero_rows, first, omega);
            else return hipErrorInvalidValue;
        case SELL_GS_OOP:
            if constexpr (std::is_same<T, double>::value) return launch_sell_mode<SELL_GS_OOP, T>(A, s_begin, s_end, x, b, y, k, ctrl, partials, n_blocks, st, zero_rows, first, omega);
            else return hipErrorInvalidValue;
        case SELL_GS_HEAD:
            if constexpr (std::is_same<T, double>::value) return launch_sell_mode<SELL_GS_HEAD, T>(A, s_begin, s_end, x, b, y, k, ctrl, partials, n_blocks, st, zero_rows, first, omega);
            else return hipErrorInvalidValue;
        case SELL_JACOBI_HEAD:
            if constexpr (std::is_same<T, double>::value) return launch_sell_mode<SELL_JACOBI_HEAD, T>(A, s_begin, s_end, x, b, y, k, ctrl, partials, n_blocks, st, zero_rows, first, omega);
            else return hipErrorInvalidValue;
        case SELL_CHEBY_HEAD:
            if constexpr (std::is_same<T, double>::value) return launch_sell_mode<SELL_CHEBY_HEAD, T>(A, s_begin, s_end, x, b, y, k, ctrl, partials, n_blocks, st, zero_rows, first, omega);
            else return hipErrorInvalidValue;
    }
    return hipErrorInvalidValue;
}

hipError_t launch_sell(SellMode mode, const SellDev& A, int s_begin, int s_end, const double* x, const double* b,
                       double* y, int k, const Ctrl* ctrl, double* partials, int* n_blocks, hipStream_t st,
                       double* zero_rows, const FirstColour* first, double omega)
{
    return launch_sell_any<double>(mode, A, s_begin, s_end, x, b, y, k, ctrl, partials, n_blocks, st, zero_rows, first, omega);
}

hipError_t launch_sell_f32(SellMode mode, const SellDev& A, int s_begin, int s_end, const float* x, const float* b,
                           float* y, int k, const Ctrl* ctrl, hipStream_t st, float* zero_rows, const FirstColour* first, double omega)
{
    if (!A.valf || mode == SELL_RESID_SS || mode == SELL_RESID_BOTH || mode >= SELL_GS_OOP) return hipErrorInvalidValue;
    return launch_sell_any<float>(mode, A, s_begin, s_end, x, b, y, k, ctrl, nullptr, nullptr, st, zero_rows, first, omega);
}

__global__ __launch_bounds__(256) void k_gershgorin(const int* a_col, const double* a_val, const int* a_slice_row, const int* a_slice_off, const int* a_slice_w,
                                                    int stride, int n_slices, unsigned long long* out)
{
    const int lane = threadIdx.x & 63, s = blockIdx.x * 4 + (threadIdx.x >> 6);
    double ratio = 0.0;
    if (s < n_slices) {
        const int row0 = a_slice_row[s], nrow = a_slice_row[s + 1] - row0, w = a_slice_w[s];
        const size_t off = (size_t)(stride ? s * stride : a_slice_off[s]) * 64 + lane;
        double sum = 0.0, diag = 0.0;
        for (int j = 0; j < w; j++) {
            const int c = a_col[off + (size_t)j * 64];
            const double v = a_val[off + (size_t)j * 64];
            if (c >= 0) { sum += fabs(v); if (c == row0 + lane) diag = v; }
        }
        if (lane < nrow && diag > 0.0) ratio = sum / diag;
    }
#pragma unroll
    for (int o = 32; o > 0; o >>= 1) ratio = fmax(ratio, __shfl_down(ratio, o, 64));
    if (lane == 0 && ratio > 0.0) atomicMax(out, (unsigned long long)__double_as_longlong(ratio));
}
hipError_t launch_gershgorin(const SellDev& A, double* out, hipStream_t st)
{
    hipError_t e = hipMemsetAsync(out, 0, sizeof(double), st);
    if (e != hipSuccess || A.n_slices <= 0) return e;
    hipLaunchKernelGGL(k_gershgorin, dim3((A.n_slices + 3) / 4), dim3(256), 0, st, A.col, A.val, A.slice_row, A.slice_off, A.slice_w, A.stride, A.n_slices,
                       (unsigned long long*)out);
    return hipGetLastError();
}


__global__ __launch_bounds__(256) void k_ss_finalize(const double* partials, int n, Ctrl* ctrl, double* out)
{
    if (ctrl->done) return;
    __shared__ double red[256];
    double s = 0.0;
    for (int i = threadIdx.x; i < n; i += 256) s += partials[i];
    red[threadIdx.x] = s;
    __syncthreads();
    for (int o = 128; o > 0; o >>= 1) {
        if ((int)threadIdx.x < o) red[threadIdx.x] += red[threadIdx.x + o];
        __syncthreads();
    }
    if (threadIdx.x == 0) *out = red[0];
}

__device__ __forceinline__ void decide_body(Ctrl* ctrl, double sumsq)
{
    const double tol = ctrl->tol;
    const double r = sqrt(sumsq);
    const int i = ctrl->n_his;
    if (i < ctrl->his_cap) ctrl->r_his[i] = r;
    ctrl->n_his = i + 1;
    ctrl->r_prev = ctrl->r_last; ctrl->r_last = r;
    if (!(r == r) || r > 1.7e308) { ctrl->status = -1; ctrl->done = 1; }
    else if (r < tol) ctrl->done = 1;
}

__global__ __launch_bounds__(256) void k_ss_finalize_decide(const double* partials, int n, Ctrl* ctrl)
{
    __shared__ double red[256];
    const int done = ctrl->done, n_his = ctrl->n_his, his_cap = ctrl->his_cap;
    const double tol = ctrl->tol;
    double* const r_his = ctrl->r_his;
    double s = 0.0;
#pragma unroll 8
    for (int i = threadIdx.x; i < n; i += 256) s += partials[i];
    if (done) return;
    red[threadIdx.x] = s;
    __syncthreads();
    for (int o = 128; o > 0; o >>= 1) {
        if ((int)threadIdx.x < o) red[threadIdx.x] += red[threadIdx.x + o];
        __syncthreads();
    }
    if (threadIdx.x == 0) {
        const double sumsq = red[0], r = sqrt(sumsq);
        ctrl->sumsq = sumsq;
        if (n_his < his_cap) r_his[n_his] = r;
        ctrl->n_his = n_his + 1;
        ctrl->r_prev = ctrl->r_last; ctrl->r_last = r;
        if (!(r == r) || r > 1.7e308) { ctrl->status = -1; ctrl->done = 1; }
        else if (r < tol) ctrl->done = 1;
    }
}

__global__ void k_decide(Ctrl* ctrl, const double* sumsq)
{
    if (ctrl->done) return;
    decide_body(ctrl, *sumsq);
}

constexpr int SS_STAGE_MIN = 16384, SS_STAGE_WGS = 128;
__global__ __launch_bounds__(256) void k_ss_stage(const double* __restrict__ partials, int n, double* __restrict__ out, const int* done)
{
    if (load_flag(done)) return;
    __shared__ double red[256];
    const int per = (n + SS_STAGE_WGS - 1) / SS_STAGE_WGS;
    const int i0 = blockIdx.x * per, i1 = min(n, i0 + per);
    double s = 0.0;
#pragma unroll 8
    for (int i = i0 + (int)threadIdx.x; i < i1; i += 256) s += partials[i];
    red[threadIdx.x] = s;
    __syncthreads();
    for (int o = 128; o > 0; o >>= 1) {
        if ((int)threadIdx.x < o) red[threadIdx.x] += red[threadIdx.x + o];
        __syncthreads();
    }
    if (threadIdx.x == 0) out[blockIdx.x] = red[0];
}
static const double* ss_stage(const double* partials, int& n, const Ctrl* ctrl, hipStream_t st)
{
    if (n < SS_STAGE_MIN) return partials;
    double* out = const_cast<double*>(partials) + n;
    hipLaunchKernelGGL(k_ss_stage, dim3(SS_STAGE_WGS), dim3(256), 0, st, partials, n, out, &ctrl->done);
    n = SS_STAGE_WGS;
    return out;
}
int ss_partials_room() { return SS_STAGE_WGS; }

hipError_t launch_ss_finalize(const double* partials, int n, Ctrl* ctrl, hipStream_t st, double* out)
{
    partials = ss_stage(partials, n, ctrl, st);
    hipLaunchKernelGGL(k_ss_finalize, dim3(1), dim3(256), 0, st, partials, n, ctrl, out ? out : &ctrl->sumsq);
    return hipGetLastError();
}
__global__ void k_decide_spec(Ctrl* ctrl, const double* sumsq)
{
    ctrl->just_done = 0;
    if (ctrl->done) return;
    decide_body(ctrl, *sumsq);
    if (ctrl->done) ctrl->just_done = 1;
}
__global__ void k_copy_unless_done(double* dst, const double* src, size_t n, const int* done)
{
    if (*done) return;
    const size_t i = (size_t)blockIdx.x * blockDim.x + threadIdx.x;
    if (i < n) dst[i] = src[i];
}
__global__ void k_restore_if_just_done(double* dst, const double* src, size_t n, const Ctrl* ctrl)
{
    if (!ctrl->just_done) return;
    const size_t i = (size_t)blockIdx.x * blockDim.x + threadIdx.x;
    if (i < n) dst[i] = src[i];
}
hipError_t launch_decide_spec(Ctrl* ctrl, const double* sumsq, hipStream_t st)
{
    hipLaunchKernelGGL(k_decide_spec, dim3(1), dim3(1), 0, st, ctrl, sumsq);
    return hipGetLastError();
}
hipError_t launch_copy_unless_done(double* dst, const double* src, size_t n, const Ctrl* ctrl, hipStream_t st)
{
// ... 751 lines not shown
}
__global__ void k_gather_vals(double* dst, const double* src, const int* map, size_t n)
{
    const size_t i = (size_t)blockIdx.x * blockDim.x + threadIdx.x;
    if (i >= n) return;
    const int m = map[i];
    if (m >= 0) dst[i] = src[m];
}
__global__ void k_scatter_dense(double* dense, const double* src, const long long* pos, int n)
{
    const int i = blockIdx.x * blockDim.x + threadIdx.x;
    if (i < n) dense[pos[i]] = src[i];
}
__global__ void k_add_at(double* v, const int* where, int n, double c)
{
    const int i = blockIdx.x * blockDim.x + threadIdx.x;
    if (i < n) v[where[i]] += c;
}
__global__ void k_dense_identity(double* dense, int np, int n)
{
    const size_t t = (size_t)blockIdx.x * blockDim.x + threadIdx.x;
    if (t >= (size_t)np * np) return;
    const int i = (int)(t / np), j = (int)(t % np);
    dense[t] = (i == j && i >= n) ? 1.0 : 0.0;
}

__global__ void k_face_terms(const double* V, const int* F, int nF, int voronoi, double* Qc, double* Qm)
{
    const int f = blockIdx.x * blockDim.x + threadIdx.x;
    if (f >= nF) return;
    const double* a = V + 3 * (size_t)F[3 * f];
    const double* b = V + 3 * (size_t)F[3 * f + 1];
    const double* c = V + 3 * (size_t)F[3 * f + 2];
    const double ux = b[0] - a[0], uy = b[1] - a[1], uz = b[2] - a[2];
    const double vx = c[0] - a[0], vy = c[1] - a[1], vz = c[2] - a[2];
    const double wx = uy * vz - uz * vy, wy = uz * vx - ux * vz, wz = ux * vy - uy * vx;
    const double dA = sqrt(wx * wx + wy * wy + wz * wz);
    double d0x = b[0] - c[0], d0y = b[1] - c[1], d0z = b[2] - c[2];
    double d1x = c[0] - a[0], d1y = c[1] - a[1], d1z = c[2] - a[2];
    double d2x = a[0] - b[0], d2y = a[1] - b[1], d2z = a[2] - b[2];
    const double l0 = sqrt(d0x * d0x + d0y * d0y + d0z * d0z);
    const double l1 = sqrt(d1x * d1x + d1y * d1y + d1z * d1z);
    const double l2 = sqrt(d2x * d2x + d2y * d2y + d2z * d2z);
    const double q0 = l0 * l0, q1 = l1 * l1, q2 = l2 * l2;
    Qc[3 * (size_t)f + 0] = (q1 + q2 - q0) / dA / 4.0;
    Qc[3 * (size_t)f + 1] = (q2 + q0 - q1) / dA / 4.0;
    Qc[3 * (size_t)f + 2] = (q0 + q1 - q2) / dA / 4.0;
    double m0, m1, m2;
    if (!voronoi) {
        m0 = m1 = m2 = dA / 6.0;
    } else {
        const double cs0 = (l2 * l2 + l1 * l1 - l0 * l0) / (l1 * l2 * 2.0);
        const double cs1 = (l0 * l0 + l2 * l2 - l1 * l1) / (l2 * l0 * 2.0);
        const double cs2 = (l1 * l1 + l0 * l0 - l2 * l2) / (l0 * l1 * 2.0);
        const double b0 = cs0 * l0, b1 = cs1 * l1, b2 = cs2 * l2;
        const double bs = b0 + b1 + b2;
        const double p0 = b0 / bs * (dA * 0.5), p1 = b1 / bs * (dA * 0.5), p2 = b2 / bs * (dA * 0.5);
        m0 = (p1 + p2) * 0.5; m1 = (p2 + p0) * 0.5; m2 = (p0 + p1) * 0.5;
        if (cs0 < 0) { m0 = 0.25 * dA; m1 = 0.125 * dA; m2 = 0.125 * dA; }
        if (cs1 < 0) { m0 = 0.125 * dA; m1 = 0.25 * dA; m2 = 0.125 * dA; }
        if (cs2 < 0) { m0 = 0.125 * dA; m1 = 0.125 * dA; m2 = 0.25 * dA; }
    }
    Qm[3 * (size_t)f + 0] = m0; Qm[3 * (size_t)f + 1] = m1; Qm[3 * (size_t)f + 2] = m2;
}
__global__ void k_mass_diag(int nV, const int* m_ptr, const int* m_idx, const double* Qm, double* Md)
{
    const int v = blockIdx.x * blockDim.x + threadIdx.x;
    if (v >= nV) return;
    double s = 0.0;
    for (int t = m_ptr[v]; t < m_ptr[v + 1]; t++) s += Qm[m_idx[t]];
    Md[v] = s;
}
__global__ void k_assemble_vals(int nnz, const int* l_ptr, const int* l_idx, const signed char* l_sgn, const double* Qc,
                                const int* diag_of, const double* Md, double mass_coef, double lap_coef, double* val, double* Lval)
{
    const int e = blockIdx.x * blockDim.x + threadIdx.x;
    if (e >= nnz) return;
    const int b = l_ptr[e], en = l_ptr[e + 1];
    double L = 0.0;
    if (b < en) {
        L = l_sgn[b] > 0 ? Qc[l_idx[b]] : -Qc[l_idx[b]];
        for (int t = b + 1; t < en; t++) L += l_sgn[t] > 0 ? Qc[l_idx[t]] : -Qc[l_idx[t]];
    }
    if (Lval) Lval[e] = L;
    const int d = diag_of[e];
    const double x = lap_coef * L;
    val[e] = d >= 0 ? mass_coef * Md[d] + x : x;
}
hipError_t launch_assemble(int nV, int nF, int nnz, const double* V, const int* F, int voronoi, const int* l_ptr, const int* l_idx,
                           const signed char* l_sgn, const int* m_ptr, const int* m_idx, const int* diag_of, double* Qc, double* Qm,
                           double* Md, double mass_coef, double lap_coef, double* val, double* Lval, hipStream_t st)
{
    hipLaunchKernelGGL(k_face_terms, dim3(grid1d(nF, 256)), dim3(256), 0, st, V, F, nF, voronoi, Qc, Qm);
    hipLaunchKernelGGL(k_mass_diag, dim3(grid1d(nV, 256)), dim3(256), 0, st, nV, m_ptr, m_idx, Qm, Md);
    hipLaunchKernelGGL(k_assemble_vals, dim3(grid1d(nnz, 256)), dim3(256), 0, st, nnz, l_ptr, l_idx, l_sgn, Qc, diag_of, Md, mass_coef, lap_coef, val, Lval);
    return hipGetLastError();
}

hipError_t launch_recipe(int n_out, const int* ptr, const int* idx, const double* coef, const double* src, double* out, hipStream_t st)
{
    if (n_out <= 0) return hipSuccess;
    hipLaunchKernelGGL(k_recipe, dim3(grid1d(n_out, 256)), dim3(256), 0, st, n_out, ptr, idx, coef, src, out);
    return hipGetLastError();
}
template <bool MAP>
__global__ __launch_bounds__(256) void k_sell_fill(const int* __restrict__ ptr, const int* __restrict__ col, const double* __restrict__ val,
                                                   const int* __restrict__ perm, const int* __restrict__ iperm, const int* __restrict__ slice_row,
                                                   const int* __restrict__ slice_off, int stride, int n_slices, int transposed, int* s_col, double* s_val, int* s_map)
{
    const int lane = threadIdx.x & 63, s = (int)blockIdx.x * 4 + (int)(threadIdx.x >> 6);
    if (s >= n_slices) return;
    const int row0 = slice_row[s], nrow = slice_row[s + 1] - row0;
    if (lane >= nrow) return;
    const int old = perm[row0 + lane];
    const int p0 = ptr[old], p1 = ptr[old + 1];
    const size_t base = (size_t)(stride ? s * stride : slice_off[s]) * 64 + lane;
    for (int p = p0; p < p1; p++) {
        const int j = col[p];
        const int c = iperm[j];
        int rank = 0;
        for (int q = p0; q < p1; q++) rank += iperm[col[q]] < c ? 1 : 0;
        int from = p;
        if (transposed) {
            int lo = ptr[j], hi = ptr[j + 1];
            while (lo < hi) { const int mid = (lo + hi) >> 1; if (col[mid] < old) lo = mid + 1; else hi = mid; }
            from = lo;
        }
        if (MAP) s_map[base + (size_t)rank * 64] = from;
        else {
            s_col[base + (size_t)rank * 64] = c;
            s_val[base + (size_t)rank * 64] = val[from];
        }
    }
}
hipError_t launch_sell_fill(const int* ptr, const int* col, const double* val, const int* perm, const int* iperm, const SellDev& S, size_t padded, hipStream_t st,
                            bool transposed)
{
    hipError_t e = hipMemsetAsync(const_cast<int*>(S.col), 0xFF, padded * sizeof(int), st);
    if (e == hipSuccess) e = hipMemsetAsync(const_cast<double*>(S.val), 0, padded * sizeof(double), st);
    if (e != hipSuccess || S.n_slices <= 0) return e;
    hipLaunchKernelGGL(k_sell_fill<false>, dim3((S.n_slices + 3) / 4), dim3(256), 0, st, ptr, col, val, perm, iperm, S.slice_row, S.slice_off, S.stride, S.n_slices,
                       transposed ? 1 : 0, const_cast<int*>(S.col), const_cast<double*>(S.val), (int*)nullptr);
    return hipGetLastError();
}
hipError_t launch_sell_fill_map(const int* ptr, const int* col, const int* perm, const int* iperm, const SellDev& S, size_t padded, bool transposed, int* map, hipStream_t st)
{
    hipError_t e = hipMemsetAsync(map, 0xFF, padded * sizeof(int), st);
    if (e != hipSuccess || S.n_slices <= 0) return e;
    hipLaunchKernelGGL(k_sell_fill<true>, dim3((S.n_slices + 3) / 4), dim3(256), 0, st, ptr, col, (const double*)nullptr, perm, iperm, S.slice_row, S.slice_off, S.stride,
                       S.n_slices, transposed ? 1 : 0, (int*)nullptr, (double*)nullptr, map);
    return hipGetLastError();
}

__global__ __launch_bounds__(256) void k_sell_diag_slots(const int* __restrict__ slice_row, const int* __restrict__ slice_off, const int* __restrict__ slice_w, int stride,
                                                         int n_slices, const int* __restrict__ s_col, int* __restrict__ slot, int* first_missing)
{
    const int lane = threadIdx.x & 63, s = (int)blockIdx.x * 4 + (int)(threadIdx.x >> 6);
    if (s >= n_slices) return;
    const int row0 = slice_row[s], nrow = slice_row[s + 1] - row0;
    if (lane >= nrow) return;
    const int r = row0 + lane, w = slice_w[s];
    const size_t base = (size_t)(stride ? s * stride : slice_off[s]) * 64 + lane;
    int at = -1;
    for (int j = 0; j < w; j++) if (s_col[base + (size_t)j * 64] == r) { at = (int)(base + (size_t)j * 64); break; }
    slot[r] = at;
    if (at < 0) atomicMin(first_missing, r);
}
hipError_t launch_sell_diag_slots(const SellDev& S, int* slot, int* first_missing, hipStream_t st)
{
    if (S.n_slices <= 0) return hipSuccess;
    hipLaunchKernelGGL(k_sell_diag_slots, dim3((S.n_slices + 3) / 4), dim3(256), 0, st, S.slice_row, S.slice_off, S.slice_w, S.stride, S.n_slices, S.col, slot, first_missing);
    return hipGetLastError();
}

__global__ void k_nothing() {}
hipError_t warm_device_code(hipStream_t st)
{
    hipLaunchKernelGGL(k_nothing, dim3(1), dim3(64), 0, st);
    return hipGetLastError();
}

__global__ __launch_bounds__(256) void k_bit_symmetric(int n, const int* __restrict__ ptr, const int* __restrict__ col, const double* __restrict__ val, int* differs)
{
    const int i = blockIdx.x * blockDim.x + threadIdx.x;
    if (i >= n) return;
    int d = 0;
    for (int p = ptr[i]; p < ptr[i + 1]; p++) {
        const int j = col[p];
        if (j < 0 || j >= n) { d |= 2; continue; }
        int lo = ptr[j], hi = ptr[j + 1];
        while (lo < hi) { const int mid = (lo + hi) >> 1; if (col[mid] < i) lo = mid + 1; else hi = mid; }
        if (lo >= ptr[j + 1] || col[lo] != i) d |= 2;
        else if (__double_as_longlong(val[lo]) != __double_as_longlong(val[p])) d |= 1;
    }
    if (d) atomicOr(differs, d);
}
hipError_t launch_bit_symmetric(int n, const int* ptr, const int* col, const double* val, int* differs, hipStream_t st)
{
    hipError_t e = hipMemsetAsync(differs, 0, sizeof(int), st);
    if (e != hipSuccess || n <= 0) return e;
    hipLaunchKernelGGL(k_bit_symmetric, dim3(grid1d((size_t)n, 256)), dim3(256), 0, st, n, ptr, col, val, differs);
    return hipGetLastError();
}

hipError_t launch_gather_vals(double* dst, const double* src, const int* map, size_t n, hipStream_t st)
{
    if (n == 0) return hipSuccess;
    hipLaunchKernelGGL(k_gather_vals, dim3(grid1d(n, 256)), dim3(256), 0, st, dst, src, map, n);
    return hipGetLastError();
}
hipError_t launch_dense_from_csr(double* dense, int np, int n, const double* src, const long long* pos, int nnz, hipStream_t st)
{
    hipLaunchKernelGGL(k_dense_identity, dim3(grid1d((size_t)np * np, 256)), dim3(256), 0, st, dense, np, n);
    if (nnz > 0) hipLaunchKernelGGL(k_scatter_dense, dim3(grid1d(nnz, 256)), dim3(256), 0, st, dense, src, pos, nnz);
    return hipGetLastError();
}
hipError_t launch_scatter_dense(double* dense, const double* src, const long long* pos, int nnz, hipStream_t st)
{
    if (nnz > 0) hipLaunchKernelGGL(k_scatter_dense, dim3(grid1d(nnz, 256)), dim3(256), 0, st, dense, src, pos, nnz);
    return hipGetLastError();
}
hipError_t launch_dense_identity(double* dense, int np, int n, hipStream_t st)
{
    hipLaunchKernelGGL(k_dense_identity, dim3(grid1d((size_t)np * np, 256)), dim3(256), 0, st, dense, np, n);
    return hipGetLastError();
}
hipError_t launch_add_at(double* v, const int* where, int n, double c, hipStream_t st)
{
    if (n <= 0) return hipSuccess;
    hipLaunchKernelGGL(k_add_at, dim3(grid1d(n, 256)), dim3(256), 0, st, v, where, n, c);
    return hipGetLastError();
}

hipError_t launch_gather_in(double* dst, const double* src, const int* map, int n, int k, int kin, int ld_src, hipStream_t st)
{
    if ((size_t)n * k == 0) return hipSuccess;
    hipLaunchKernelGGL(k_gather_in, dim3(grid1d((size_t)n * kin, 256)), dim3(256), 0, st, dst, src, map, n, k, kin, ld_src);
    return hipGetLastError();
}
hipError_t launch_scatter_out(double* dst, const double* src, const int* map, int n, int k, int kin, int ld_dst, hipStream_t st)
{
    if ((size_t)n * k == 0) return hipSuccess;
    hipLaunchKernelGGL(k_scatter_out, dim3(grid1d((size_t)n * k, 256)), dim3(256), 0, st, dst, src, map, n, k, kin, ld_dst);
    return hipGetLastError();
}
hipError_t launch_scatter_cm(double* dst, const double* src, const int* idx, int n, int k, int ld_src, int ld_dst,
                             hipStream_t st)
{
    if ((size_t)n * k == 0) return hipSuccess;
    hipLaunchKernelGGL(k_scatter_cm, dim3(grid1d((size_t)n * k, 256)), dim3(256), 0, st, dst, src, idx, n, k, ld_src, ld_dst);
    return hipGetLastError();
}
hipError_t launch_gather_cm(double* dst, const double* src, const int* idx, int n, int k, int ld_src, int ld_dst,
                            hipStream_t st)
{
    if ((size_t)n * k == 0) return hipSuccess;
    hipLaunchKernelGGL(k_gather_cm, dim3(grid1d((size_t)n * k, 256)), dim3(256), 0, st, dst, src, idx, n, k, ld_src, ld_dst);
    return hipGetLastError();
}
hipError_t launch_csr_sub(int n_rows, const int* ptr, const int* col, const double* val, const double* x, int ldx,
                          double* y, int ld, int k, hipStream_t st)
{
    if ((size_t)n_rows * k == 0) return hipSuccess;
    hipLaunchKernelGGL(k_csr_sub, dim3(grid1d((size_t)n_rows * k, 256)), dim3(256), 0, st, n_rows, ptr, col, val, x, ldx, y, ld, k);
    return hipGetLastError();
}

}
```

### surface_multigrid_code_amd/csrc/smg_device.hpp

```cpp
#pragma once
#include <hip/hip_runtime_api.h>

#include <cstdint>

namespace smg {

struct Ctrl {
    int done;
    int n_his;
    int status;
    int just_done;
    double sumsq;
    double tol;
    double* r_his;
    int his_cap;
    int pad_;
    double r_last, r_prev;
};

struct SellDev {
    int n_rows = 0, n_cols = 0, n_slices = 0;
    int C = 64;
    const int* slice_row = nullptr;
    const int* slice_off = nullptr;
    const int* slice_w = nullptr;
    int stride = 0;
    int w_lo = 0;
    int w_max = 0;
    const int* order = nullptr;
    const int* col = nullptr;
    const double* val = nullptr;
    const float* valf = nullptr;
    int long_n = 0;
    const int* long_row = nullptr;
    const int* long_ptr = nullptr;
    const int* long_col = nullptr;
    const double* long_val = nullptr;
    const float* long_valf = nullptr;
};

enum SellMode {
    SELL_AX = 0,
    SELL_RESID = 1,
    SELL_RESID_SS = 2,
    SELL_ADD = 3,
    SELL_GS = 4,
    SELL_RESID_BOTH = 5,
    SELL_JACOBI = 6,
    SELL_CHEBY = 7,
    SELL_GS_OOP = 8,
    SELL_GS_HEAD = 9,
    SELL_JACOBI_HEAD = 10,
    SELL_CHEBY_HEAD = 11,
};
constexpr bool sell_is_gs(int m) { return m == SELL_GS || m == SELL_GS_OOP || m == SELL_GS_HEAD; }
constexpr bool sell_is_oop(int m) { return m == SELL_GS_OOP || m == SELL_GS_HEAD; }
constexpr bool sell_is_jacobi(int m) { return m == SELL_JACOBI || m == SELL_JACOBI_HEAD; }
constexpr bool sell_is_cheby(int m) { return m == SELL_CHEBY || m == SELL_CHEBY_HEAD; }
constexpr bool sell_is_head(int m) { return m == SELL_GS_HEAD || m == SELL_JACOBI_HEAD || m == SELL_CHEBY_HEAD; }
constexpr bool sell_has_ss(int m) { return sell_is_head(m) || m == SELL_RESID_SS || m == SELL_RESID_BOTH; }

struct FirstColour {
    const int* diag_slot = nullptr;
    int n_first = 0;
    const double* val = nullptr;
    const float* valf = nullptr;
    int jacobi = 0;
    double omega = 1.0;
    double* d = nullptr;
    float* df = nullptr;
    double c1 = 0.0;
};
hipError_t launch_sell(SellMode mode, const SellDev& A, int s_begin, int s_end, const double* x, const double* b,
                       double* y, int k, const Ctrl* ctrl, double* partials, int* n_blocks, hipStream_t st,
                       double* zero_rows = nullptr, const FirstColour* first = nullptr, double omega = 1.0);
hipError_t launch_sell_f32(SellMode mode, const SellDev& A, int s_begin, int s_end, const float* x, const float* b,
                           float* y, int k, const Ctrl* ctrl, hipStream_t st, float* zero_rows = nullptr,
                           const FirstColour* first = nullptr, double omega = 1.0);
hipError_t launch_gershgorin(const SellDev& A, double* out, hipStream_t st);
struct Bsr3Dev {
    int n_vert = 0, n_slices = 0, w_max = 0;
    const int* slice_row = nullptr;
    const int* slice_off = nullptr;
    const int* slice_w = nullptr;
    const int* order = nullptr;
    const int* col = nullptr;
    const double* val = nullptr;
    const float* valf = nullptr;
};
hipError_t launch_bsr3(SellMode mode, const Bsr3Dev& A, int s_begin, int s_end, const double* x, const double* b, double* y, int k, const Ctrl* ctrl,
                       double* partials, int* n_blocks, hipStream_t st, double omega = 1.0, double c1 = 0.0, double* dvec = nullptr);
hipError_t launch_bsr3_f32(SellMode mode, const Bsr3Dev& A, int s_begin, int s_end, const float* x, const float* b, float* y, int k, const Ctrl* ctrl, hipStream_t st,
                           double omega = 1.0, double c1 = 0.0, float* dvec = nullptr);
hipError_t launch_bsr3_gershgorin(const Bsr3Dev& A, double* out, hipStream_t st);
int bsr3_blocks(int n_slices);
hipError_t launch_bsr3_fill(const int* ptr, const int* col, const double* val, const int* gptr, const int* gcol, const int* perm, const int* iperm, const Bsr3Dev& B,
                            size_t panel_cols, bool transposed, hipStream_t st);

struct BgsDev {
    int n_blocks = 0, n_colors = 0, xrows = 0;
    const int* hdr = nullptr;
    const int* xrow = nullptr;
    const int* ugrow = nullptr;
    const int* ulrow = nullptr;
    const double* udiag = nullptr;
    const int* eidx = nullptr;
    const double* eval = nullptr;
};
hipError_t launch_bgs(const BgsDev& P, int b_begin, int b_end, const double* b, double* u, int k, const Ctrl* ctrl, hipStream_t st);

struct WgsDev {
    int n_pieces = 0, n_colors = 0, rim_pitch = 0, nb_max = 0;
    const int* hdr = nullptr;
    const int* grow = nullptr;
    const int* meta = nullptr;
    const double* diag = nullptr;
    const int* rim = nullptr;
    const unsigned* eoff = nullptr;
    const double* eval = nullptr;
};
hipError_t launch_wgs(const WgsDev& P, int q_begin, int q_end, const double* b, double* u, int k, const Ctrl* ctrl, hipStream_t st);

struct UnionDev {
    int m = 0, his_cap = 0, max_rows = 0;
    const int* rows = nullptr;
    const int* rptr = nullptr;
    const int* crow_member = nullptr;
    const long long* moff = nullptr;
    const int* mlda = nullptr;
    const int* mrow0 = nullptr;
    double* ss = nullptr;
    double* his = nullptr;
    int* nhis = nullptr;
    int* done = nullptr;
    double* zsave = nullptr;
};
hipError_t launch_blockdiag_gemv_add(const UnionDev& U, const double* Ainv, int n, const double* b, double* u, int k, const Ctrl* ctrl, hipStream_t st);
hipError_t launch_union_sumsq_decide(const UnionDev& U, const double* r, const double* u, int k, Ctrl* ctrl, hipStream_t st);
hipError_t launch_union_restore(const UnionDev& U, double* u, int k, const Ctrl* ctrl, hipStream_t st);
hipError_t launch_scatter_dense(double* dense, const double* src, const long long* pos, int nnz, hipStream_t st);
hipError_t launch_dense_identity(double* dense, int np, int n, hipStream_t st);

struct TiledDev {
    int n_tiles = 0, nc = 0, P = 0, sweeps = 0, max_ext = 0, w_max = 0, threads = 512;
    const int* hdr = nullptr;
    const int* ext_rows = nullptr;
    const int* pcol = nullptr;
    const double* pval = nullptr;
    const int* prow = nullptr;
    const double* pdiag = nullptr;
};
hipError_t launch_tiled_gs(const TiledDev& T, const double* x, const double* b, double* y, int k, const Ctrl* ctrl, hipStream_t st);
hipError_t tiled_gs_prepare(int max_ext);

struct SparseCholDev {
    int n = 0;
    const int* perm = nullptr;
    const int *rptr = nullptr, *rcol = nullptr;
    const int *cptr = nullptr, *crow = nullptr;
    const double *rval = nullptr, *cval = nullptr, *diag = nullptr;
    double* work = nullptr;
    int* err = nullptr;
};
hipError_t launch_sparse_coarse_solve(const SparseCholDev& F, const double* b, double* u, int k, const Ctrl* ctrl, hipStream_t st);
int sparse_coarse_work_cols(int k);

constexpr int SCHUR_M_MAX_DEV = 128;
struct SchurDev {
    int n = 0, nb = 0, ns = 0, ns_pad = 0;
    const int *irow = nullptr, *bsize = nullptr, *srow = nullptr, *sptr = nullptr, *sidx = nullptr, *aptr = nullptr, *ablk = nullptr, *apan = nullptr;
    double* arena = nullptr;
    float* arena32 = nullptr;
    long long off_D = 0, off_P = 0, off_W = 0, off_S = 0, off_C = 0;
    const long long *coff = nullptr, *pos = nullptr, *pos2 = nullptr, *ones = nullptr, *rdst = nullptr, *rdst2 = nullptr, *rsrc = nullptr;
    const int* rptr = nullptr;
    int nnz = 0, n_ones = 0, n_red = 0;
    double *g = nullptr, *xs = nullptr;
    float *g32 = nullptr, *xs32 = nullptr;
    double* sym_work = nullptr;
    double* gj_work = nullptr;
};
hipError_t launch_schur_factor(const SchurDev& F, const double* vals, hipStream_t st);
hipError_t launch_schur_check(const SchurDev& F, int* d_flag, hipStream_t st);
hipError_t launch_schur_solve(const SchurDev& F, const double* b, double* u, int k, const Ctrl* ctrl, hipStream_t st);
hipError_t launch_schur_solve_f32(const SchurDev& F, const float* b, float* u, int k, const Ctrl* ctrl, hipStream_t st);

int sell_blocks(int n_slices);
int sell_wide_blocks(int n_slices, int k);

int ss_partials_room();
hipError_t launch_ss_finalize(const double* partials, int n, Ctrl* ctrl, hipStream_t st, double* out = nullptr);
hipError_t launch_decide(Ctrl* ctrl, const double* sumsq, hipStream_t st);
hipError_t launch_decide_spec(Ctrl* ctrl, const double* sumsq, hipStream_t st);
hipError_t launch_copy_unless_done(double* dst, const double* src, size_t n, const Ctrl* ctrl, hipStream_t st);
hipError_t launch_restore_if_just_done(double* dst, const double* src, size_t n, const Ctrl* ctrl, hipStream_t st);
hipError_t launch_ss_finalize_decide(const double* partials, int n, Ctrl* ctrl, hipStream_t st);

hipError_t launch_dense_gemv_add(const double* Ainv, int n, int lda, const double* b, double* u, int k, int ld,
                                 const Ctrl* ctrl, hipStream_t st, double* sym_work = nullptr);
hipError_t launch_dense_gemv_add_f32(const float* Ainv, int n, int lda, const float* b, float* u, int k, int ld,
                                     const Ctrl* ctrl, hipStream_t st, float* sym_work = nullptr);
hipError_t launch_sym_gemv_tiles(const double* Ainv, int lda, const double* b, double* part, hipStream_t st);
hipError_t launch_sym_gemv_tiles_f32(const float* Ainv, int lda, const float* b, float* part, hipStream_t st);
hipError_t launch_cvt_f64_f32(float* dst, const double* src, size_t n, hipStream_t st);
hipError_t launch_residual_to_f32(float* b32, float* u32, const double* r64, size_t n, const Ctrl* ctrl, hipStream_t st);
hipError_t launch_add_correction(double* z, const float* e, size_t n, const Ctrl* ctrl, hipStream_t st);
hipError_t launch_spd_inverse(double* M, int n, double* work, hipStream_t st);

hipError_t launch_recipe(int n_out, const int* ptr, const int* idx, const double* coef, const double* src, double* out, hipStream_t st);
hipError_t launch_sell_fill(const int* ptr, const int* col, const double* val, const int* perm, const int* iperm, const SellDev& S, size_t padded, hipStream_t st,
                            bool transposed = false);
hipError_t launch_sell_diag_slots(const SellDev& S, int* slot, int* first_missing, hipStream_t st);
hipError_t warm_device_code(hipStream_t st);
hipError_t launch_sell_fill_map(const int* ptr, const int* col, const int* perm, const int* iperm, const SellDev& S, size_t padded, bool transposed, int* map, hipStream_t st);
hipError_t launch_bit_symmetric(int n, const int* ptr, const int* col, const double* val, int* differs, hipStream_t st);
hipError_t launch_gather_vals(double* dst, const double* src, const int* map, size_t n, hipStream_t st);
hipError_t launch_dense_from_csr(double* dense, int np, int n, const double* src, const long long* pos, int nnz, hipStream_t st);
hipError_t launch_add_at(double* v, const int* where, int n, double c, hipStream_t st);

hipError_t launch_assemble(int nV, int nF, int nnz, const double* V, const int* F, int voronoi, const int* l_ptr, const int* l_idx,
                           const signed char* l_sgn, const int* m_ptr, const int* m_idx, const int* diag_of, double* Qc, double* Qm,
                           double* Md, double mass_coef, double lap_coef, double* val, double* Lval, hipStream_t st);

hipError_t launch_gather_in(double* dst, const double* src, const int* map, int n, int k, int kin, int ld_src,
                            hipStream_t st);
hipError_t launch_scatter_out(double* dst, const double* src, const int* map, int n, int k, int kin, int ld_dst,
                              hipStream_t st);
hipError_t launch_scatter_cm(double* dst, const double* src, const int* idx, int n, int k, int ld_src, int ld_dst,
                             hipStream_t st);
hipError_t launch_gather_cm(double* dst, const double* src, const int* idx, int n, int k, int ld_src, int ld_dst,
                            hipStream_t st);
hipError_t launch_csr_sub(int n_rows, const int* ptr, const int* col, const double* val, const double* x, int ldx,
                          double* y, int ld, int k, hipStream_t st);

}
```

### surface_multigrid_code_amd/csrc/smg_hier.hpp

```cpp
#pragma once
#include <memory>
#include <hip/hip_runtime_api.h>

#include <atomic>
#include <cstdint>
#include <string>
#include <vector>

#include "smg_bsr3.hpp"
#include "smg_coarse.hpp"
#include "smg_device.hpp"
#include "smg_mesh.hpp"
#include "smg_order.hpp"
#include "smg_sparse.hpp"
#include "smg_tiled.hpp"
#include "smg_bgs.hpp"
#include "smg_wgs.hpp"
#include "smg_schur.hpp"

namespace smg {

inline std::atomic<long long>& devbuf_live_bytes() { static std::atomic<long long> v{0}; return v; }

template <typename T>
struct PinBuf {
    T* p = nullptr;
    size_t n = 0;
    PinBuf() = default;
    PinBuf(const PinBuf&) = delete;
    PinBuf& operator=(const PinBuf&) = delete;
    ~PinBuf() { release(); }
    void release() { if (p) (void)hipHostFree(p); p = nullptr; n = 0; }
    hipError_t ensure(size_t count)
    {
        if (count <= n) return hipSuccess;
        release();
        hipError_t e = hipHostMalloc((void**)&p, count * sizeof(T), hipHostMallocDefault);
        if (e == hipSuccess) n = count; else p = nullptr;
        return e;
    }
};

template <typename T>
struct DevBuf {
    T* p = nullptr;
    size_t n = 0;
    DevBuf() = default;
    DevBuf(const DevBuf&) = delete;
    DevBuf& operator=(const DevBuf&) = delete;
    DevBuf(DevBuf&& o) noexcept : p(o.p), n(o.n) { o.p = nullptr; o.n = 0; }
    DevBuf& operator=(DevBuf&& o) noexcept { if (this != &o) { release(); p = o.p; n = o.n; o.p = nullptr; o.n = 0; } return *this; }
    ~DevBuf() { release(); }
    void release() { if (p) { (void)hipFree(p); devbuf_live_bytes() -= (long long)(n * sizeof(T)); } p = nullptr; n = 0; }
    hipError_t alloc(size_t count)
    {
        release();
        if (count == 0) return hipSuccess;
        hipError_t e = hipMalloc((void**)&p, count * sizeof(T));
        if (e == hipSuccess) { n = count; devbuf_live_bytes() += (long long)(count * sizeof(T)); } else p = nullptr;
        return e;
    }
    hipError_t ensure(size_t count) { return count <= n ? hipSuccess : alloc(count); }
    template <class Alloc>
    hipError_t upload(const std::vector<T, Alloc>& v)
    {
        hipError_t e = alloc(v.size());
        if (e != hipSuccess || v.empty()) return e;
        return hipMemcpy(p, v.data(), v.size() * sizeof(T), hipMemcpyHostToDevice);
    }
    template <class Alloc>
    hipError_t upload_in_place(const std::vector<T, Alloc>& v, bool* moved)
    {
        if (p && v.size() == n) return v.empty() ? hipSuccess : hipMemcpy(p, v.data(), v.size() * sizeof(T), hipMemcpyHostToDevice);
        *moved = true;
        return upload(v);
    }
};

struct SellBuf {
    DevBuf<int> slice_row, slice_off, slice_w, col, order;
    DevBuf<double> val;
    SellDev view;
    std::vector<int> color_slice_ptr;
    DevBuf<int> diag_slot;
    int n_first = 0;
    int n_all = 0;
    long stored = 0, padded = 0, used = 0;
    hipError_t upload(const Sell& S);
    DevBuf<int> long_row, long_ptr, long_col;
    DevBuf<double> long_val;
    DevBuf<float> long_valf;
    hipError_t upload_long(const std::vector<int>& rows, const std::vector<int>& ptr, const std::vector<int>& col, const std::vector<double>& val);
};

struct Bsr3Buf {
    DevBuf<int> slice_row, slice_off, slice_w, col, order;
    DevBuf<double> val;
    DevBuf<float> valf;
    Bsr3Dev view;
    std::vector<int> color_slice_ptr;
    long stored = 0, blocks = 0, padded = 0;
    hipError_t upload(const Bsr3Sell& S);
};

struct TiledBuf {
    DevBuf<int> hdr, ext_rows, pcol, prow, map, mapd;
    DevBuf<double> pval, pdiag;
    TiledDev view;
    long updates = 0;
    std::vector<int> host_map, host_mapd;
    bool tried = false;
};

struct BgsBuf {
    DevBuf<int> hdr, xrow, ugrow, ulrow, eidx, map, mapd;
    DevBuf<double> eval, udiag;
    BgsDev view;
    std::vector<int> color_ptr;
    std::vector<int> host_map, host_mapd;
    std::vector<int> host_rows, host_blk_ptr;
    double rim = 0.0, fill = 0.0;
    bool tried = false;
};

struct WgsBuf {
    DevBuf<int> hdr, grow, meta, rim, map, mapd;
    DevBuf<unsigned> eoff;
    DevBuf<double> eval, diag;
    WgsDev view;
    std::vector<int> color_ptr;
    std::vector<int> host_map, host_mapd;
    std::vector<int> host_rows, host_piece_ptr;
    double rim_ratio = 0.0, phases_mean = 0.0;
    int phases_max = 0;
    bool tried = false;
};

struct Level {
    std::vector<double> V;
    std::vector<int> F;
    Csr P_full;
    std::shared_ptr<DecimationLog> dec_log;
    Csr A;
    std::vector<double> A_diag;
    Csr P, PT;
    Ordering ord;
    uint64_t ord_key = 0;
    Csr A_int, P_int, PT_int;
    Ordering vord;
    Csr Pv, PTv;
    Bsr3Buf bA, bAT;
    DevBuf<int> mapB, mapBT;
    SellBuf dA, dP, dPT;
    SellBuf dAT;
    bool gs_on_transpose = false;
    bool P_device_filled = false, PT_device_filled = false;
    bool device_filled = false;
    Csr vpat;
    bool A_bit_symmetric = false;
    TiledBuf tiled[4];
    WgsBuf wgs;
    BgsBuf bgs;
    std::vector<int> A_int_src;
    DevBuf<double> d_Aval;
    DevBuf<double> d_Tval;
    DevBuf<int> mapA, mapAT;
    DevBuf<int> r1_ptr, r1_idx, r2_ptr, r2_idx;
    DevBuf<double> r1_coef, r2_coef;
    int nnzT = 0;
    DevBuf<float> a32, at32, p32, pt32;
    SellDev dA32, dAT32, dP32, dPT32;
    DevBuf<float> b32, u32, r32;
    DevBuf<double> b, u, r;
    DevBuf<double> t;
    DevBuf<float> t32;
    DevBuf<double> d;
    DevBuf<float> d32;
    double lam = 0.0;
    int n = 0;
};

struct GraphKey {
    int k = 0, k_user = 0, pre = 0, post = 0, precision = 0, smoother = 0, jacobi_max_rows = 0;
    double omega = 0.0, cheby_fraction = 0.0;
    bool head_fuse = false;
    bool operator==(const GraphKey& o) const
    {
        return k == o.k && k_user == o.k_user && pre == o.pre && post == o.post && precision == o.precision && smoother == o.smoother &&
               jacobi_max_rows == o.jacobi_max_rows && omega == o.omega && cheby_fraction == o.cheby_fraction && head_fuse == o.head_fuse;
    }
    bool operator!=(const GraphKey& o) const { return !(*this == o); }
};

struct ProfScope { std::string name; long count = 0; double ms = 0.0; };
struct ProfRec { int scope; hipEvent_t e0, e1; };

}

struct smg_hierarchy {
    int n_levels = 0;
    std::vector<smg::Level> lv;
    int n_full = 0;
    bool has_known = false, precomputed = false;
    std::vector<int> known, unknown;
    smg::Csr LHS_unused;
    smg::Csr Auk;
    smg::DevBuf<int> d_map0;
    smg::DevBuf<int> d_perm0;
    smg::DevBuf<int> d_unknown, d_known;
    smg::DevBuf<int> d_auk_ptr, d_auk_col;
    smg::DevBuf<double> d_auk_val;
    uint64_t pre_key = 0;
    int p_version = 0;
    bool input_canonical = false;
    bool recipes_built = false, host_stale = false;
    int nnz_input = 0;
    std::vector<int> lhs_src, auk_src;
    smg::DevBuf<int> d_lhs_src, d_auk_src, d_diag_idx;
    smg::DevBuf<long long> d_dense_pos;
    smg::DevBuf<double> d_Afull;
    struct EarlyUpload { smg::DevBuf<int> ptr, col; smg::DevBuf<double> val; bool valid = false; } early0;
    int nc = 0, nc_pad = 0;
    smg::DevBuf<double> d_Ainv;
    smg::DevBuf<float> d_Ainv32;
    smg::DevBuf<double> d_sympart;
    bool coarse_sparse = false;
    int coarse_dense_max = 16384;
    bool coarse_dense_max_user = false;
    bool mem_lean = false;
    int wgs_mode = -1;
    int bgs_min_rows = -1;
    smg::SparseChol chol;
    smg::DevBuf<int> c_perm, c_rptr, c_rcol, c_cptr, c_crow, c_err;
    smg::DevBuf<double> c_rval, c_cval, c_diag, c_work;
    smg::SparseCholDev c_view;
    bool coarse_schur = false;
    int coarse_schur_when = 2;
    int coarse_schur_min = 2048;
    int coarse_schur_big = 6144;
    int coarse_schur_max = 65536;
    bool schur_declined = false;
    smg::SchurPlan schur;
    struct SchurBuf {
        smg::DevBuf<int> irow, bsize, srow, sptr, sidx, aptr, ablk, acol, rptr;
        smg::DevBuf<long long> coff, pos, pos2, ones, rdst, rdst2, rsrc;
// ... 62 lines not shown
```

### surface_multigrid_code_amd/csrc/smg_precompute.cpp

```cpp
#include <hip/hip_runtime.h>

#include <algorithm>
#include <atomic>
#include <chrono>
#include <condition_variable>
#include <mutex>
#include <cmath>
#include <cstdarg>
#include <cstdio>
#include <cstdlib>
#include <cstring>
#include <exception>
#include <functional>
#include <memory>
#include <numeric>
#include <string>
#include <thread>
#include <vector>

#include "smg_internal.hpp"

using namespace smg;

static bool bit_symmetric(const Csr& A)
// ... 670 lines not shown
                h->c_perm.release(); h->c_rptr.release(); h->c_rcol.release(); h->c_cptr.release(); h->c_crow.release(); h->c_rval.release(); h->c_cval.release(); h->c_diag.release(); h->c_work.release();
            }
            h->d_Ainv.release(); h->d_Ainv32.release(); h->d_sympart.release();
            return SMG_OK;
        }
    }
    h->sch.release(); h->schur = SchurPlan();
    if (Lc.n > h->coarse_dense_max) {
        h->nc = Lc.n; h->nc_pad = Lc.n;
        return coarse_factor_sparse(h, Lc.A, false);
    }
    h->coarse_sparse = false;
    h->nc = nc; h->nc_pad = np;
    std::vector<long long> pos((size_t)Lc.A.nnz());
    for (int i = 0; i < nc; i++)
        for (int p = Lc.A.ptr[i]; p < Lc.A.ptr[i + 1]; p++) pos[(size_t)p] = (long long)i * np + Lc.A.col[p];
    DevBuf<long long> d_pos;
    DevBuf<double> d_val;
    HIPCHK(d_pos.upload(pos));
    HIPCHK(d_val.upload(Lc.A.val));
    HIPCHK(h->d_Ainv.ensure((size_t)np * np));
    HIPCHK(launch_dense_from_csr(h->d_Ainv.p, np, nc, d_val.p, d_pos.p, (int)Lc.A.nnz(), h->stream));
    if (env_int("SMG_SYM_COARSE", 1)) HIPCHK(h->d_sympart.ensure((size_t)(np / 64) * (np / 64) * 64)); else h->d_sympart.release();
    DevBuf<double> work;
    HIPCHK(work.alloc((size_t)2 * np * 64 + 2 * 64 * 64));
    HIPCHK(launch_spd_inverse(h->d_Ainv.p, np, work.p, h->stream));
    HIPCHK(hipStreamSynchronize(h->stream));
    return SMG_OK;
}

static int level_images(smg_hierarchy* h, int lv, int sym0)
{
    const int L = h->n_levels;
    const int sellC = SELL_C;
    const bool region = env_int("SMG_REGION_ORDER", 1) != 0;
    const bool blk = h->bs == 3;
    const int lp = lv + 1;
    Level& Lw = h->lv[lv];
    Level& Lp = h->lv[lp];
    {
        std::vector<std::function<void()>> tasks;
        tasks.push_back([h, lv, &Lw] {
            Lw.device_filled = false;
            if (device_fill_candidate(h, lv)) {
                Lw.A_int = Csr(); Lw.A_int_src.clear();
                Lw.device_filled = true;
            } else Lw.A_int = permute(Lw.A, Lw.ord.perm, Lw.ord.perm, &Lw.A_int_src);
        });
        tasks.push_back([h, &Lw, &Lp] {
            Lp.P_device_filled = device_fill_rows(h, Lp.P.nr);
            if (Lp.P_device_filled) Lp.P_int = Csr(); else Lp.P_int = permute(Lp.P, Lw.ord.perm, Lp.ord.perm);
        });
        tasks.push_back([h, &Lw, &Lp] {
            static const int long_min = env_int("SMG_LONG_ROW_MIN", 65);
            bool ok = device_fill_rows(h, Lp.PT.nr);
            if (ok && long_min > 0) for (int r = 0; r < Lp.PT.nr && ok; r++) if (Lp.PT.ptr[(size_t)r + 1] - Lp.PT.ptr[(size_t)r] >= long_min) ok = false;
            Lp.PT_device_filled = ok;
            if (ok) Lp.PT_int = Csr(); else Lp.PT_int = permute(Lp.PT, Lp.ord.perm, Lw.ord.perm);
        });
        run_image_tasks("operators in the device numbering", lv, tasks);
    }
    int bad = 0;
    hipError_t eA = hipSuccess, eT = hipSuccess, eP = hipSuccess, eQ = hipSuccess;
    std::vector<std::function<void()>> tasks;
    tasks.push_back([&] {
        DeviceScope ds(h->device);
        if (blk && Lw.device_filled) {
            Lw.dA = SellBuf();
            DeviceCsr D;
            eA = D.put(Lw.A, lv == 0 && !h->has_known ? &h->early0 : nullptr);
            int differs = sym0 == 1 ? 0 : -1;
            DevBuf<int> d_differs, d_gptr, d_gcol, d_perm, d_iperm;
            if (eA == hipSuccess && differs < 0) {
                eA = d_differs.alloc(1);
                if (eA == hipSuccess) eA = launch_bit_symmetric(Lw.A.nr, D.ptr, D.col, D.val, d_differs.p, h->aux[0]);
                if (eA == hipSuccess) eA = hipMemcpyAsync(&differs, d_differs.p, sizeof(int), hipMemcpyDeviceToHost, h->aux[0]);
                if (eA == hipSuccess) eA = hipStreamSynchronize(h->aux[0]);
            }
            if (eA != hipSuccess) return;
            if (Lw.A.nr != Lw.A.nc || (differs & 2)) { bad = 1; return; }
            Lw.A_bit_symmetric = differs == 0;
            Lw.gs_on_transpose = differs != 0;
            Lw.bAT = Bsr3Buf(); Lw.dAT = SellBuf();
            const Csr& G = Lw.vpat;
            const std::vector<int>& vp = Lw.vord.perm;
            std::vector<int> row_len(vp.size());
            parallel_for((long)vp.size(), 1 << 16, [&](long r0, long r1) { for (long r = r0; r < r1; r++) row_len[(size_t)r] = G.ptr[(size_t)vp[(size_t)r] + 1] - G.ptr[(size_t)vp[(size_t)r]]; });
            if (eA == hipSuccess) eA = d_gptr.upload(G.ptr);
            if (eA == hipSuccess) eA = d_gcol.upload(G.col);
            if (eA == hipSuccess) eA = d_perm.upload(vp);
            if (eA == hipSuccess) eA = d_iperm.upload(Lw.vord.iperm);
            const Bsr3Sell S = bsr3_layout(row_len, &Lw.vord.color_ptr, region, Lw.A.nnz(), G.nnz());
            if (eA == hipSuccess) eA = Lw.bA.upload(S);
            if (eA == hipSuccess) eA = launch_bsr3_fill(D.ptr, D.col, D.val, d_gptr.p, d_gcol.p, d_perm.p, d_iperm.p, Lw.bA.view, (size_t)S.slice_off.back(), false, h->aux[0]);
            if (eA == hipSuccess && Lw.gs_on_transpose) {
                const Bsr3Sell ST = bsr3_layout(row_len, &Lw.vord.color_ptr, false, Lw.A.nnz(), G.nnz());
                eT = Lw.bAT.upload(ST);
                if (eT == hipSuccess) eT = launch_bsr3_fill(D.ptr, D.col, D.val, d_gptr.p, d_gcol.p, d_perm.p, d_iperm.p, Lw.bAT.view, (size_t)ST.slice_off.back(), true, h->aux[0]);
            }
            if (eA == hipSuccess) eA = hipStreamSynchronize(h->aux[0]);
            return;
        }
        if (blk) {
            Lw.dA = SellBuf();
            Bsr3Sell S = build_bsr3(Lw.A_int, &Lw.vord.color_ptr, region, false);
            eA = Lw.bA.upload(S);
            return;
        }
        Lw.bA = Bsr3Buf();
        if (Lw.device_filled) {
            DeviceCsr D;
            eA = D.put(Lw.A, lv == 0 && !h->has_known ? &h->early0 : nullptr);
            int differs = sym0 == 1 ? 0 : -1;
            if (eA == hipSuccess && differs < 0) {
                DevBuf<int> d_differs;
                eA = d_differs.alloc(1);
                if (eA == hipSuccess) eA = launch_bit_symmetric(Lw.A.nr, D.ptr, D.col, D.val, d_differs.p, h->aux[0]);
                if (eA == hipSuccess) eA = hipMemcpyAsync(&differs, d_differs.p, sizeof(int), hipMemcpyDeviceToHost, h->aux[0]);
                if (eA == hipSuccess) eA = hipStreamSynchronize(h->aux[0]);
            }
            if (eA != hipSuccess) return;
            if (Lw.A.nr != Lw.A.nc || (differs & 2)) { bad = 1; return; }
            Lw.A_bit_symmetric = differs == 0;
            Lw.gs_on_transpose = differs != 0;
            Lw.dAT = SellBuf(); Lw.bAT = Bsr3Buf();
            eA = device_fill_sell(Lw.dA, Lw.A, D, Lw.ord.perm, Lw.ord.iperm, &Lw.ord.color_ptr, region, h->aux[0], false, h->mem_lean ? 0 : -1);
            if (eA == hipSuccess && Lw.gs_on_transpose) eT = device_fill_sell(Lw.dAT, Lw.A, D, Lw.ord.perm, Lw.ord.iperm, &Lw.ord.color_ptr, false, h->aux[0], true, h->mem_lean ? 0 : -1);
            return;
        }
        Sell S = build_sell(Lw.A_int, &Lw.ord.color_ptr, sellC, region, h->mem_lean ? 0 : -1);
        eA = Lw.dA.upload(S);
    });
    tasks.push_back([&] {
        DeviceScope ds(h->device);
        if (Lw.device_filled) return;
        Lw.dAT = SellBuf();
        Lw.bAT = Bsr3Buf();
        if (Lw.A_int.nnz() >= (1L << 22) && bit_symmetric(Lw.A_int)) { Lw.gs_on_transpose = false; return; }
        Csr AT = transpose(Lw.A_int);
        Lw.gs_on_transpose = !(AT.ptr == Lw.A_int.ptr && AT.col == Lw.A_int.col && AT.val == Lw.A_int.val);
        if (Lw.gs_on_transpose) {
            if (!(AT.ptr == Lw.A_int.ptr && AT.col == Lw.A_int.col)) { bad = 1; return; }
            if (blk) { Bsr3Sell S = build_bsr3(AT, &Lw.vord.color_ptr, false, false); eT = Lw.bAT.upload(S); }
            else { Sell S = build_sell(AT, &Lw.ord.color_ptr, sellC, false, h->mem_lean ? 0 : -1); eT = Lw.dAT.upload(S); }
        }
    });
    static const bool tr_region = env_int("SMG_TRANSFER_REGION_ORDER", 1) != 0;
    tasks.push_back([&] {
        DeviceScope ds(h->device);
        const Ordering& Of = blk ? Lw.vord : Lw.ord;
        const bool cut = tr_region && region && Of.color_ptr.size() > 2;
        if (!blk && Lp.P_device_filled) {
            eP = device_fill_sell(Lp.dP, Lp.P, Of.perm, Lp.ord.iperm, cut ? &Of.color_ptr : nullptr, cut, h->aux[1], h->mem_lean ? 0 : -1);
            return;
        }
        Csr Pvi;
        if (blk) Pvi = permute(Lp.Pv, Of.perm, Lp.vord.perm);
        Sell S = build_sell(blk ? Pvi : Lp.P_int, cut ? &Of.color_ptr : nullptr, sellC, cut, h->mem_lean ? 0 : -1);
        eP = Lp.dP.upload(S);
    });
    tasks.push_back([&] {
        DeviceScope ds(h->device);
        const Ordering& Oc = blk ? Lp.vord : Lp.ord;
        const bool cut = tr_region && region && lp < L - 1 && Oc.color_ptr.size() > 2;
        static const int long_min = env_int("SMG_LONG_ROW_MIN", 65);
        if (!blk && Lp.PT_device_filled) {
            eQ = device_fill_sell(Lp.dPT, Lp.PT, Oc.perm, Lw.ord.iperm, cut ? &Oc.color_ptr : nullptr, cut, h->aux[2], h->mem_lean ? 0 : -1);
            if (eQ == hipSuccess) eQ = Lp.dPT.upload_long({}, {0}, {}, {});
            return;
        }
        Csr PTvi;
        if (blk) PTvi = permute(Lp.PTv, Oc.perm, Lw.vord.perm);
        const Csr& M = blk ? PTvi : Lp.PT_int;
        std::vector<int> lrow, lptr{0}, lcol;
        std::vector<double> lval;
        if (long_min > 0)
            for (int r = 0; r < M.nr; r++)
                if (M.ptr[r + 1] - M.ptr[r] >= long_min) {
                    lrow.push_back(r);
                    lcol.insert(lcol.end(), M.col.begin() + M.ptr[r], M.col.begin() + M.ptr[r + 1]);
                    lval.insert(lval.end(), M.val.begin() + M.ptr[r], M.val.begin() + M.ptr[r + 1]);
                    lptr.push_back((int)lcol.size());
                }
        if (lrow.empty()) {
            Sell S = build_sell(M, cut ? &Oc.color_ptr : nullptr, sellC, cut, h->mem_lean ? 0 : -1);
            eQ = Lp.dPT.upload(S);
            if (eQ == hipSuccess) eQ = Lp.dPT.upload_long(lrow, lptr, lcol, lval);
            return;
        }
        Csr Ms;
        Ms.nr = M.nr; Ms.nc = M.nc; Ms.ptr.assign((size_t)M.nr + 1, 0);
        {
            size_t li = 0;
            for (int r = 0; r < M.nr; r++) {
                const bool is_long = li < lrow.size() && lrow[li] == r;
                if (is_long) li++;
                else { Ms.col.insert(Ms.col.end(), M.col.begin() + M.ptr[r], M.col.begin() + M.ptr[r + 1]); Ms.val.insert(Ms.val.end(), M.val.begin() + M.ptr[r], M.val.begin() + M.ptr[r + 1]); }
                Ms.ptr[(size_t)r + 1] = (int)Ms.col.size();
            }
        }
        Sell S = build_sell(Ms, cut ? &Oc.color_ptr : nullptr, sellC, cut, h->mem_lean ? 0 : -1);
        eQ = Lp.dPT.upload(S);
        if (eQ == hipSuccess) eQ = Lp.dPT.upload_long(lrow, lptr, lcol, lval);
    });
    run_image_tasks("images", lv, tasks);
    if (bad) return fail(SMG_ERR_INVALID, "level %d matrix is not structurally symmetric", lv);
    HIPCHK(eA); HIPCHK(eT); HIPCHK(eP); HIPCHK(eQ);
    return SMG_OK;
}

static int finish_images(smg_hierarchy* h)
{
    const Level& L0 = h->lv[0];
    std::vector<int> map0((size_t)L0.n);
    for (int i = 0; i < L0.n; i++) map0[(size_t)i] = h->has_known ? h->unknown[(size_t)L0.ord.perm[(size_t)i]] : L0.ord.perm[(size_t)i];
    HIPCHK(h->d_map0.upload(map0));
    HIPCHK(h->d_perm0.upload(L0.ord.perm));
    if (h->has_known) {
        HIPCHK(h->d_unknown.upload(h->unknown));
        HIPCHK(h->d_known.upload(h->known));
        HIPCHK(h->d_auk_ptr.upload(h->Auk.ptr));
        HIPCHK(h->d_auk_col.upload(h->Auk.col));
        HIPCHK(h->d_auk_val.upload(h->Auk.val));
    }
    h->lam_valid = false;
    return SMG_OK;
}


static uint64_t precompute_key(const smg_hierarchy* h, int n, const int* rowptr, const int* col, const int* known, int n_known)
{
    uint64_t key = 1469598103934665603ull;
    const int hdr[4] = {n, n_known, h->p_version, h->n_levels};
    key = fnv_mix(key, hdr, 4);
    key = fnv_mix(key, rowptr, (size_t)n + 1);
    key = fnv_mix(key, col, (size_t)rowptr[n]);
    if (known) key = fnv_mix(key, known, (size_t)n_known);
    return key ? key : 1;
}

static int build_recipes(smg_hierarchy* h)
{
    const int L = h->n_levels;
    const int sellC = SELL_C;
    HIPCHK(hipStreamSynchronize(h->stream));
    if (h->bs == 3) for (int lv = 0; lv < L; lv++) { int rc = ensure_A_int(h, lv); if (rc) return rc; }
    for (hipStream_t& a : h->aux) if (!a) HIPCHK(hipStreamCreateWithFlags(&a, hipStreamNonBlocking));
    drop_graphs(h);
    drop_tiled(h);
    std::vector<int> bad(L, 0);
    std::vector<hipError_t> errs((size_t)2 * L, hipSuccess);
    StageTimer tm;
    {
        std::vector<std::function<void()>> tasks;
        auto up = [](hipError_t& acc, hipError_t e) { if (acc == hipSuccess) acc = e; };
        for (int lv = 0; lv < L; lv++) {
            if (lv < L - 1) tasks.push_back([&, lv] {
                DeviceScope ds(h->device);
                Level& Lv = h->lv[lv];
                hipError_t& er = errs[2 * lv];
                if (h->bs != 3) {
                    up(er, Lv.d_Aval.upload(Lv.A.val));
                    DevBuf<int> d_ptr, d_col, d_perm, d_iperm;
                    up(er, d_ptr.upload(Lv.A.ptr)); up(er, d_col.upload(Lv.A.col)); up(er, d_perm.upload(Lv.ord.perm)); up(er, d_iperm.upload(Lv.ord.iperm));
                    hipStream_t st2 = h->aux[lv % 3];
                    up(er, Lv.mapA.alloc((size_t)Lv.dA.padded));
                    if (er == hipSuccess) up(er, launch_sell_fill_map(d_ptr.p, d_col.p, d_perm.p, d_iperm.p, Lv.dA.view, (size_t)Lv.dA.padded, false, Lv.mapA.p, st2));
                    if (!Lv.gs_on_transpose && er == hipSuccess) {
                        DeviceCsr D;
                        D.ptr = d_ptr.p; D.col = d_col.p; D.val = Lv.d_Aval.p;
                        up(er, device_fill_sell(Lv.dAT, Lv.A, D, Lv.ord.perm, Lv.ord.iperm, &Lv.ord.color_ptr, false, st2, true, h->mem_lean ? 0 : -1));
                        Lv.gs_on_transpose = true;
                    }
                    up(er, Lv.mapAT.alloc((size_t)Lv.dAT.padded));
                    if (er == hipSuccess) up(er, launch_sell_fill_map(d_ptr.p, d_col.p, d_perm.p, d_iperm.p, Lv.dAT.view, (size_t)Lv.dAT.padded, true, Lv.mapAT.p, st2));
                    if (er == hipSuccess) up(er, hipStreamSynchronize(st2));
                    return;
                }
                std::vector<int> m;
                std::vector<int> tsrc;
                Csr AT = transpose(Lv.A_int, &tsrc);
                if (!(AT.ptr == Lv.A_int.ptr && AT.col == Lv.A_int.col)) { bad[lv] = 1; return; }
                if (h->bs == 3) {
                    {
                        Bsr3Sell S = build_bsr3(Lv.A_int, &Lv.vord.color_ptr, false);
                        m.resize(S.entry.size());
                        for (size_t i = 0; i < S.entry.size(); i++) m[i] = S.entry[i] >= 0 ? Lv.A_int_src[S.entry[i]] : -1;
                    }
                    up(er, Lv.mapB.upload(m));
                    Bsr3Sell ST = build_bsr3(AT, &Lv.vord.color_ptr, false);
                    m.resize(ST.entry.size());
                    for (size_t i = 0; i < ST.entry.size(); i++) m[i] = ST.entry[i] >= 0 ? Lv.A_int_src[tsrc[ST.entry[i]]] : -1;
                    up(er, Lv.mapBT.upload(m));
                    if (!Lv.gs_on_transpose) { up(er, Lv.bAT.upload(ST)); Lv.gs_on_transpose = true; }
                    return;
                }
                {
                    Sell S = build_sell(Lv.A_int, &Lv.ord.color_ptr, sellC, false, h->mem_lean ? 0 : -1);
                    m.resize(S.entry.size());
                    for (size_t i = 0; i < S.entry.size(); i++) m[i] = S.entry[i] >= 0 ? Lv.A_int_src[S.entry[i]] : -1;
                }
                up(er, Lv.mapA.upload(m));
                Sell ST = build_sell(AT, &Lv.ord.color_ptr, sellC, false, h->mem_lean ? 0 : -1);
                m.resize(ST.entry.size());
                for (size_t i = 0; i < ST.entry.size(); i++) m[i] = ST.entry[i] >= 0 ? Lv.A_int_src[tsrc[ST.entry[i]]] : -1;
                up(er, Lv.mapAT.upload(m));
                if (!Lv.gs_on_transpose) { up(er, Lv.dAT.upload(ST)); Lv.gs_on_transpose = true; }
            });
            tasks.push_back([&, lv] {
                DeviceScope ds(h->device);
                Level& Lv = h->lv[lv];
                hipError_t& er = errs[2 * lv + 1];
                if (h->bs == 3 || lv == L - 1) up(er, Lv.d_Aval.upload(Lv.A.val));
                if (lv == 0) return;
                const Csr& Af = h->lv[lv - 1].A;
                Csr T = spgemm(Lv.PT, Af);
                Recipe r;
                spgemm_recipe(Lv.PT, Af, true, T, r);
                up(er, Lv.r1_ptr.upload(r.ptr)); up(er, Lv.r1_idx.upload(r.idx)); up(er, Lv.r1_coef.upload(r.coef));
                spgemm_recipe(T, Lv.P, false, Lv.A, r);
                up(er, Lv.r2_ptr.upload(r.ptr)); up(er, Lv.r2_idx.upload(r.idx)); up(er, Lv.r2_coef.upload(r.coef));
                Lv.nnzT = (int)T.nnz();
                up(er, Lv.d_Tval.alloc(T.nnz()));
            });
        }
        parallel_tasks(tasks);
    }
    for (int lv = 0; lv < L; lv++)
        if (bad[lv]) return fail(SMG_ERR_INVALID, "level %d matrix is not structurally symmetric", lv);
    for (hipError_t e : errs) HIPCHK(e);
    tm.lap("recipes: host work + uploads");
    {
        const Level& Lc = h->lv[L - 1];
        std::vector<long long> pos(Lc.A.nnz());
        std::vector<int> dg;
        for (int i = 0; i < Lc.n; i++)
            for (int p = Lc.A.ptr[i]; p < Lc.A.ptr[i + 1]; p++) {
                pos[p] = (long long)i * h->nc_pad + Lc.A.col[p];
                if (Lc.A.col[p] == i) dg.push_back(p);
            }
// ... 300 lines not shown
```

Baseline: 3309 V-cycles/s.

## Encode transfer-operator values as 2-bit codes packed into column indices

When a prolongation or restriction SELL matrix has at most four distinct values, as with midpoint-subdivision transfers, the values are packed as a 2-bit code into the low bits of each column index and the fp64/fp32 value arrays are dropped. The SpMV kernels for the AX and ADD modes get a CODED template variant that decodes the value from a four-entry table, so the transfer operators stop reading 8 bytes of value per nonzero. This adds a host scan, an encode kernel and a sync at setup, and the decode costs a few extra integer operations per nonzero.

```diff
diff --git a/surface_multigrid_code_amd/csrc/smg_capi.cpp b/surface_multigrid_code_amd/csrc/smg_capi.cpp
--- a/surface_multigrid_code_amd/csrc/smg_capi.cpp
+++ b/surface_multigrid_code_amd/csrc/smg_capi.cpp
@@ -144,6 +144,7 @@
     view.n_rows = S.n_rows; view.n_cols = S.n_cols; view.n_slices = S.n_slices; view.C = S.C;
     view.order = S.region_order.empty() ? nullptr : order.p;
     view.slice_row = slice_row.p; view.slice_off = slice_off.p; view.slice_w = slice_w.p; view.col = col.p; view.val = val.p;
+    view.codes = 0;
     view.stride = S.stride; view.w_lo = S.w_lo;
     view.w_max = 0;
     for (int w : S.slice_w) view.w_max = std::max(view.w_max, w);
@@ -192,6 +193,36 @@
     if ((e = long_col.upload(col)) != hipSuccess) return e;
     if ((e = long_val.upload(val)) != hipSuccess) return e;
     view.long_n = (int)rows.size(); view.long_row = long_row.p; view.long_ptr = long_ptr.p; view.long_col = long_col.p; view.long_val = long_val.p;
+    return hipSuccess;
+}
+
+hipError_t SellBuf::encode_codes(const double* vals, size_t n_vals, hipStream_t st)
+{
+    static const bool on = env_int("SMG_TRANSFER_CODES", 1) != 0;
+    if (!on || view.codes || view.long_n > 0 || padded == 0 || !view.val || view.n_cols >= (1 << 29)) return hipSuccess;
+    double tab[4] = {0.0, 0.0, 0.0, 0.0};
+    int n_tab = 0;
+    for (size_t p = 0; p < n_vals; p++) {
+        const double v = vals[p];
+        int i = 0;
+        while (i < n_tab && std::memcmp(&tab[i], &v, sizeof v) != 0) i++;
+        if (i == n_tab) { if (n_tab == 4) return hipSuccess; tab[n_tab++] = v; }
+    }
+    if (n_tab == 0) return hipSuccess;
+    DevBuf<int> ccol, d_bad;
+    hipError_t e = ccol.alloc((size_t)padded);
+    if (e == hipSuccess) e = d_bad.alloc(1);
+    if (e == hipSuccess) e = hipMemsetAsync(d_bad.p, 0, sizeof(int), st);
+    if (e == hipSuccess) e = launch_sell_encode(view, (size_t)padded, tab, n_tab, ccol.p, d_bad.p, st);
+    int bad = 1;
+    if (e == hipSuccess) e = hipMemcpyAsync(&bad, d_bad.p, sizeof(int), hipMemcpyDeviceToHost, st);
+    if (e == hipSuccess) e = hipStreamSynchronize(st);
+    if (e != hipSuccess || bad) return e;
+    col = std::move(ccol);
+    val.release();
+    view.col = col.p; view.val = nullptr; view.valf = nullptr;
+    view.codes = 1;
+    for (int i = 0; i < 4; i++) { view.tab[i] = tab[i]; view.tabf[i] = (float)tab[i]; }
     return hipSuccess;
 }
 
diff --git a/surface_multigrid_code_amd/csrc/smg_cycle.cpp b/surface_multigrid_code_amd/csrc/smg_cycle.cpp
--- a/surface_multigrid_code_amd/csrc/smg_cycle.cpp
+++ b/surface_multigrid_code_amd/csrc/smg_cycle.cpp
@@ -347,7 +347,7 @@
                 src.view.long_valf = src.long_valf.p;
             }
             view = src.view;
-            if (src.padded == 0) { view.valf = nullptr; return SMG_OK; }
+            if (src.padded == 0 || src.view.codes) { view.valf = nullptr; return SMG_OK; }
             HIPCHK(dst.ensure((size_t)src.padded));
             HIPCHK(launch_cvt_f64_f32(dst.p, src.view.val, (size_t)src.padded, h->stream));
             view.valf = dst.p;
diff --git a/surface_multigrid_code_amd/csrc/smg_device.hip b/surface_multigrid_code_amd/csrc/smg_device.hip
--- a/surface_multigrid_code_amd/csrc/smg_device.hip
+++ b/surface_multigrid_code_amd/csrc/smg_device.hip
@@ -19,9 +19,14 @@
 }
 
 
-template <typename T> struct CoarseInit { T* u; const T* gs_val; const int* diag_slot; int n_first; int jacobi; T omega; T* d; T c1; };
-
-template <int MODE, int KB, typename T, int W0C = -1, int WPB = 4>
+template <typename T> struct CoarseInit { T* u; const T* gs_val; const int* diag_slot; int n_first; int jacobi; T omega; T* d; T c1; int codes; T tab[4]; };
+template <typename T> __device__ __forceinline__ T code_val(const CoarseInit<T>& z, int cw)
+{
+    const T lo = (cw & 1) ? z.tab[1] : z.tab[0], hi = (cw & 1) ? z.tab[3] : z.tab[2];
+    return (cw & 2) ? hi : lo;
+}
+
+template <int MODE, int KB, typename T, int W0C = -1, int WPB = 4, bool CODED = false>
 __global__ __launch_bounds__(64 * WPB) void k_sell(const int* a_col, const T* a_val, const int* a_order, const int* a_slice_off, int a_stride,
                                               int a_w_lo, int s_begin, int s_end, int n_blocks, int use_order, const T* x,
                                               const int* a_slice_row, const int* a_slice_w, const T* b, T* y, int ld, const int* done,
@@ -45,13 +50,13 @@
         const int W0 = W0C >= 0 ? W0C : (A.w_lo < 8 ? A.w_lo : 8);
         const int off0 = (W0C >= 0 || A.stride) ? s * A.stride : A.slice_off[s];
         const int* cp = A.col + (size_t)off0 * C + lane;
-        const T* vp = a_val + (size_t)off0 * C + lane;
+        const T* vp = CODED ? nullptr : a_val + (size_t)off0 * C + lane;
         constexpr int U = W0C > 8 ? W0C : 8;
         int c0[U];
         T v0[U];
 #pragma unroll
         for (int t = 0; t < U; t++) {
-            if (t < W0) { c0[t] = cp[(size_t)t * C]; v0[t] = vp[(size_t)t * C]; }
+            if (t < W0) { c0[t] = cp[(size_t)t * C]; v0[t] = CODED ? (T)0 : vp[(size_t)t * C]; }
             else { c0[t] = -1; v0[t] = (T)0; }
         }
         {
@@ -83,7 +88,14 @@
             else bv[q] = live ? b[(size_t)rowb * ld + q] : (T)0;
             if (CHEB && live && z.c1 != (T)0) dold[q] = z.d[(size_t)rowb * ld + q];
         }
-        auto consume = [&](const int (&c)[U], const T (&v)[U]) {
+        auto consume = [&](const int (&cw)[U], const T (&vw)[U]) {
+            int c[U];
+            T v[U];
+#pragma unroll
+            for (int t = 0; t < U; t++) {
+                if constexpr (CODED) { c[t] = cw[t] >> 2; v[t] = code_val<T>(z, cw[t]); }
+                else { c[t] = cw[t]; v[t] = vw[t]; }
+            }
             T xv[U][KB];
             T xo[MODE == SELL_GS_HEAD ? U : 1][KB];
 #pragma unroll
@@ -124,7 +136,7 @@
             T v[U];
 #pragma unroll
             for (int t = 0; t < U; t++) {
-                if ((j0 + t) < w) { c[t] = cp[(size_t)(j0 + t) * C]; v[t] = vp[(size_t)(j0 + t) * C]; }
+                if ((j0 + t) < w) { c[t] = cp[(size_t)(j0 + t) * C]; v[t] = CODED ? (T)0 : vp[(size_t)(j0 + t) * C]; }
                 else { c[t] = -1; v[t] = (T)0; }
             }
             consume(c, v);
@@ -199,7 +211,7 @@
             for (int t = bt * 8; t < bt * 8 + 8; t++) {
                 const int tt = t < w ? t : w - 1;
                 c[t] = cp[(size_t)tt * C];
-                v[t] = vp[(size_t)tt * C];
+                v[t] = z.codes ? 0.0 : vp[(size_t)tt * C];
             }
         } else {
 #pragma unroll
@@ -210,6 +222,10 @@
     if (MODE == SELL_AX && live && rowb < z.n_first) zd = z.gs_val[z.diag_slot[rowb]];
 #pragma unroll
     for (int q = 0; q < KB; q++) bv[q] = (MODE == SELL_RESID && live) ? b[(size_t)rowb * ld + q] : 0.0;
+    if (z.codes) {
+#pragma unroll
+        for (int t = 0; t < S; t++) { v[t] = code_val<double>(z, c[t]); c[t] >>= 2; }
+    }
     double xv[S][KB];
 #pragma unroll
     for (int t = 0; t < S; t++) {
@@ -310,7 +326,7 @@
                     const int e = q * 64 + lane, tt = e / RW, rr = e % RW;
                     const bool in2 = e < U * RW && (j0 + tt) < w;
                     cL[q] = in2 ? cp[(size_t)(j0 + tt) * 64 + sub * RW + rr] : -1;
-                    vL[q] = in2 ? vp[(size_t)(j0 + tt) * 64 + sub * RW + rr] : (T)0;
+                    vL[q] = (in2 && !z.codes) ? vp[(size_t)(j0 + tt) * 64 + sub * RW + rr] : (T)0;
                 }
             }
 #pragma unroll
@@ -321,12 +337,13 @@
                     (void)in;
                     if constexpr (G == 1) {
                         cc[t][r] = in ? cp[(size_t)(j0 + t) * 64 + rl[r]] : -1;
-                        vv[t][r] = in ? vp[(size_t)(j0 + t) * 64 + rl[r]] : (T)0;
+                        vv[t][r] = (in && !z.codes) ? vp[(size_t)(j0 + t) * 64 + rl[r]] : (T)0;
                     } else {
                         const int src = t * RW + r * G + g;
                         cc[t][r] = __shfl(cL[(t * RW + r * G) / 64], src & 63, 64);
                         vv[t][r] = __shfl(vL[(t * RW + r * G) / 64], src & 63, 64);
                     }
+                    if (z.codes) { vv[t][r] = code_val<T>(z, cc[t][r]); cc[t][r] >>= 2; }
                 }
 #pragma unroll
             for (int t = 0; t < U; t++)
@@ -487,6 +504,15 @@
 }
 template <> const double* host_vals<double>(const SellDev& A) { return A.val; }
 template <> const float* host_vals<float>(const SellDev& A) { return A.valf; }
+template <typename T> static CoarseInit<T> coarse_codes(const SellDev& A, T* zero_rows, int c0, const FirstColour* first, double omega)
+{
+    CoarseInit<T> z = coarse_init<T>(zero_rows, c0, first, omega);
+    z.codes = A.codes;
+    for (int i = 0; i < 4; i++) {
+        if constexpr (std::is_same<T, double>::value) z.tab[i] = A.tab[i]; else z.tab[i] = A.tabf[i];
+    }
+    return z;
+}
 
 static long wide_latency_max()
 {
@@ -528,6 +554,39 @@
 static constexpr int sell_wpb() { return 4; }
 static int gs_wpb() { static const int v = getenv("SMG_GS_WPB") ? atoi(getenv("SMG_GS_WPB")) : 4; return v; }
 int sell_blocks(int n_slices) { return (n_slices + sell_wpb() - 1) / sell_wpb(); }
+
+template <int MODE, typename T, bool CODED>
+static void launch_narrow(const SellDev& A, int kb, int nb, int ns, int grid, int nbarg, bool one_xcd, int s_begin, int s_end, int use_order, const T* xx,
+                          const T* bb, T* yy, int k, const int* done, double* pp, const CoarseInit<T>& zz, hipStream_t st)
+{
+    switch (kb) {
+        case 1: {
+            const int w0 = A.stride > 0 ? (A.w_lo < 8 ? A.w_lo : 8) : -1;
+            static const int pitch_env = getenv("SMG_PITCH_SPEC_MAX") ? atoi(getenv("SMG_PITCH_SPEC_MAX")) : -1;
+            const int pitch_max = pitch_env >= 0 ? pitch_env : (sell_is_gs(MODE) ? 32 : 64);
+            if (nb <= pitch_max && A.stride == 12 && w0 >= 7) hipLaunchKernelGGL((k_sell<MODE, 1, T, 12, 4, CODED>), dim3(grid), dim3(64 * sell_wpb()), 0, st, A.col, CODED ? nullptr : host_vals<T>(A), A.order, A.slice_off, A.stride, A.w_lo, s_begin, s_end, nbarg, use_order, xx, A.slice_row, A.slice_w, bb, yy, k, done, pp, zz);
+            else if (!CODED && w0 == 7 && MODE == SELL_GS && !one_xcd && gs_wpb() == 8) hipLaunchKernelGGL((k_sell<MODE == SELL_GS ? MODE : SELL_GS, 1, T, 7, 8>), dim3((ns + 7) / 8), dim3(512), 0, st, A.col, CODED ? nullptr : host_vals<T>(A), A.order, A.slice_off, A.stride, A.w_lo, s_begin, s_end, (ns + 7) / 8, use_order, xx, A.slice_row, A.slice_w, bb, yy, k, done, pp, zz);
+            else if (!CODED && w0 == 7 && MODE == SELL_GS && !one_xcd && gs_wpb() == 2) hipLaunchKernelGGL((k_sell<MODE == SELL_GS ? MODE : SELL_GS, 1, T, 7, 2>), dim3((ns + 1) / 2), dim3(128), 0, st, A.col, CODED ? nullptr : host_vals<T>(A), A.order, A.slice_off, A.stride, A.w_lo, s_begin, s_end, (ns + 1) / 2, use_order, xx, A.slice_row, A.slice_w, bb, yy, k, done, pp, zz);
+            else if (w0 == 7) hipLaunchKernelGGL((k_sell<MODE, 1, T, 7, 4, CODED>), dim3(grid), dim3(64 * sell_wpb()), 0, st, A.col, CODED ? nullptr : host_vals<T>(A), A.order, A.slice_off, A.stride, A.w_lo, s_begin, s_end, nbarg, use_order, xx, A.slice_row, A.slice_w, bb, yy, k, done, pp, zz);
+            else if (w0 == 8) hipLaunchKernelGGL((k_sell<MODE, 1, T, 8, 4, CODED>), dim3(grid), dim3(64 * sell_wpb()), 0, st, A.col, CODED ? nullptr : host_vals<T>(A), A.order, A.slice_off, A.stride, A.w_lo, s_begin, s_end, nbarg, use_order, xx, A.slice_row, A.slice_w, bb, yy, k, done, pp, zz);
+            else if (w0 == 2) hipLaunchKernelGGL((k_sell<MODE, 1, T, 2, 4, CODED>), dim3(grid), dim3(64 * sell_wpb()), 0, st, A.col, CODED ? nullptr : host_vals<T>(A), A.order, A.slice_off, A.stride, A.w_lo, s_begin, s_end, nbarg, use_order, xx, A.slice_row, A.slice_w, bb, yy, k, done, pp, zz);
+            else hipLaunchKernelGGL((k_sell<MODE, 1, T, -1, 4, CODED>), dim3(grid), dim3(64 * sell_wpb()), 0, st, A.col, CODED ? nullptr : host_vals<T>(A), A.order, A.slice_off, A.stride, A.w_lo, s_begin, s_end, nbarg, use_order, xx, A.slice_row, A.slice_w, bb, yy, k, done, pp, zz);
+            break;
+        }
+        case 2:
+            if (A.stride > 0 && A.w_lo == 7) hipLaunchKernelGGL((k_sell<MODE, 2, T, 7, 4, CODED>), dim3(grid), dim3(64 * sell_wpb()), 0, st, A.col, CODED ? nullptr : host_vals<T>(A), A.order, A.slice_off, A.stride, A.w_lo, s_begin, s_end, nbarg, use_order, xx, A.slice_row, A.slice_w, bb, yy, k, done, pp, zz);
+            else hipLaunchKernelGGL((k_sell<MODE, 2, T, -1, 4, CODED>), dim3(grid), dim3(64 * sell_wpb()), 0, st, A.col, CODED ? nullptr : host_vals<T>(A), A.order, A.slice_off, A.stride, A.w_lo, s_begin, s_end, nbarg, use_order, xx, A.slice_row, A.slice_w, bb, yy, k, done, pp, zz);
+            break;
+        case 3:
+            if (A.stride > 0 && A.w_lo == 7) hipLaunchKernelGGL((k_sell<MODE, 3, T, 7, 4, CODED>), dim3(grid), dim3(64 * sell_wpb()), 0, st, A.col, CODED ? nullptr : host_vals<T>(A), A.order, A.slice_off, A.stride, A.w_lo, s_begin, s_end, nbarg, use_order, xx, A.slice_row, A.slice_w, bb, yy, k, done, pp, zz);
+            else hipLaunchKernelGGL((k_sell<MODE, 3, T, -1, 4, CODED>), dim3(grid), dim3(64 * sell_wpb()), 0, st, A.col, CODED ? nullptr : host_vals<T>(A), A.order, A.slice_off, A.stride, A.w_lo, s_begin, s_end, nbarg, use_order, xx, A.slice_row, A.slice_w, bb, yy, k, done, pp, zz);
+            break;
+        default:
+            if (A.stride > 0 && A.w_lo == 7) hipLaunchKernelGGL((k_sell<MODE, 4, T, 7, 4, CODED>), dim3(grid), dim3(64 * sell_wpb()), 0, st, A.col, CODED ? nullptr : host_vals<T>(A), A.order, A.slice_off, A.stride, A.w_lo, s_begin, s_end, nbarg, use_order, xx, A.slice_row, A.slice_w, bb, yy, k, done, pp, zz);
+            else hipLaunchKernelGGL((k_sell<MODE, 4, T, -1, 4, CODED>), dim3(grid), dim3(64 * sell_wpb()), 0, st, A.col, CODED ? nullptr : host_vals<T>(A), A.order, A.slice_off, A.stride, A.w_lo, s_begin, s_end, nbarg, use_order, xx, A.slice_row, A.slice_w, bb, yy, k, done, pp, zz);
+            break;
+    }
+}
 
 template <int MODE, typename T>
 static hipError_t launch_sell_mode(const SellDev& A, int s_begin, int s_end_in, const T* x, const T* b, T* y,
@@ -554,7 +613,7 @@
             const T* bb = b ? b + c0 : nullptr;
             T* yy = y ? y + c0 : nullptr;
             double* pp = partials ? partials + poff : nullptr;
-            const CoarseInit<T> zz = coarse_init<T>(zero_rows, c0, first, omega);
+            const CoarseInit<T> zz = coarse_codes<T>(A, zero_rows, c0, first, omega);
             int wnb = 0;
             switch (kw) {
                 case 64: launch_wide_one<MODE, 64, T>(A, s_begin, s_end, use_order, xx, bb, yy, k, done, pp, zz, st, &wnb); break;
@@ -575,7 +634,7 @@
         const T* bb = b ? b + c0 : nullptr;
         T* yy = y ? y + c0 : nullptr;
         double* pp = partials ? partials + poff : nullptr;
-        const CoarseInit<T> zz = coarse_init<T>(zero_rows, c0, first, omega);
+        const CoarseInit<T> zz = coarse_codes<T>(A, zero_rows, c0, first, omega);
         poff += (size_t)nb;
         if constexpr (std::is_same<T, double>::value && (MODE == SELL_AX || MODE == SELL_RESID)) {
             int kd = kb;
@@ -585,7 +644,7 @@
                     int kk = kb - cc;
                     while (kk > 1 && !deep_wanted(MODE, A.w_max, kk)) kk--;
                     const int nbm = A.w_max <= 24 ? 3 : A.w_max <= 40 ? 5 : 8;
-                    const CoarseInit<T> zc = coarse_init<T>(zero_rows, c0 + cc, first, omega);
+                    const CoarseInit<T> zc = coarse_codes<T>(A, zero_rows, c0 + cc, first, omega);
 #define SMG_DEEP_LAUNCH(KB, NB) hipLaunchKernelGGL((k_sell_deep<MODE, KB, NB>), dim3(nb), dim3(256), 0, st, A.col, A.val, A.order, A.slice_off, A.stride, s_begin, s_end, nb, use_order, \
                                                    xx ? xx + cc : nullptr, A.slice_row, A.slice_w, bb ? bb + cc : nullptr, yy + cc, k, done, zc)
                     if (nbm == 3) { if (kk == 1) SMG_DEEP_LAUNCH(1, 3); else if (kk == 2) SMG_DEEP_LAUNCH(2, 3); else SMG_DEEP_LAUNCH(3, 3); }
@@ -597,36 +656,13 @@
                 continue;
             }
         }
-        switch (kb) {
-            case 1: {
-                const int w0 = A.stride > 0 ? (A.w_lo < 8 ? A.w_lo : 8) : -1;
-                static const int pitch_env = getenv("SMG_PITCH_SPEC_MAX") ? atoi(getenv("SMG_PITCH_SPEC_MAX")) : -1;
-                const int pitch_max = pitch_env >= 0 ? pitch_env : (sell_is_gs(MODE) ? 32 : 64);
-                if (nb <= pitch_max && A.stride == 12 && w0 >= 7) hipLaunchKernelGGL((k_sell<MODE, 1, T, 12>), dim3(grid), dim3(64 * sell_wpb()), 0, st, A.col, host_vals<T>(A), A.order, A.slice_off, A.stride, A.w_lo, s_begin, s_end, nbarg, use_order, xx, A.slice_row, A.slice_w, bb, yy, k, done, pp, zz);
-                else if (w0 == 7 && MODE == SELL_GS && !one_xcd && gs_wpb() == 8) hipLaunchKernelGGL((k_sell<MODE == SELL_GS ? MODE : SELL_GS, 1, T, 7, 8>), dim3((ns + 7) / 8), dim3(512), 0, st, A.col, host_vals<T>(A), A.order, A.slice_off, A.stride, A.w_lo, s_begin, s_end, (ns + 7) / 8, use_order, xx, A.slice_row, A.slice_w, bb, yy, k, done, pp, zz);
-                else if (w0 == 7 && MODE == SELL_GS && !one_xcd && gs_wpb() == 2) hipLaunchKernelGGL((k_sell<MODE == SELL_GS ? MODE : SELL_GS, 1, T, 7, 2>), dim3((ns + 1) / 2), dim3(128), 0, st, A.col, host_vals<T>(A), A.order, A.slice_off, A.stride, A.w_lo, s_begin, s_end, (ns + 1) / 2, use_order, xx, A.slice_row, A.slice_w, bb, yy, k, done, pp, zz);
-                else if (w0 == 7) hipLaunchKernelGGL((k_sell<MODE, 1, T, 7>), dim3(grid), dim3(64 * sell_wpb()), 0, st, A.col, host_vals<T>(A), A.order, A.slice_off, A.stride, A.w_lo, s_begin, s_end, nbarg, use_order, xx, A.slice_row, A.slice_w, bb, yy, k, done, pp, zz);
-                else if (w0 == 8) hipLaunchKernelGGL((k_sell<MODE, 1, T, 8>), dim3(grid), dim3(64 * sell_wpb()), 0, st, A.col, host_vals<T>(A), A.order, A.slice_off, A.stride, A.w_lo, s_begin, s_end, nbarg, use_order, xx, A.slice_row, A.slice_w, bb, yy, k, done, pp, zz);
-                else if (w0 == 2) hipLaunchKernelGGL((k_sell<MODE, 1, T, 2>), dim3(grid), dim3(64 * sell_wpb()), 0, st, A.col, host_vals<T>(A), A.order, A.slice_off, A.stride, A.w_lo, s_begin, s_end, nbarg, use_order, xx, A.slice_row, A.slice_w, bb, yy, k, done, pp, zz);
-                else hipLaunchKernelGGL((k_sell<MODE, 1, T>), dim3(grid), dim3(64 * sell_wpb()), 0, st, A.col, host_vals<T>(A), A.order, A.slice_off, A.stride, A.w_lo, s_begin, s_end, nbarg, use_order, xx, A.slice_row, A.slice_w, bb, yy, k, done, pp, zz);
-                break;
-            }
-            case 2:
-                if (A.stride > 0 && A.w_lo == 7) hipLaunchKernelGGL((k_sell<MODE, 2, T, 7>), dim3(grid), dim3(64 * sell_wpb()), 0, st, A.col, host_vals<T>(A), A.order, A.slice_off, A.stride, A.w_lo, s_begin, s_end, nbarg, use_order, xx, A.slice_row, A.slice_w, bb, yy, k, done, pp, zz);
-                else hipLaunchKernelGGL((k_sell<MODE, 2, T>), dim3(grid), dim3(64 * sell_wpb()), 0, st, A.col, host_vals<T>(A), A.order, A.slice_off, A.stride, A.w_lo, s_begin, s_end, nbarg, use_order, xx, A.slice_row, A.slice_w, bb, yy, k, done, pp, zz);
-                break;
-            case 3:
-                if (A.stride > 0 && A.w_lo == 7) hipLaunchKernelGGL((k_sell<MODE, 3, T, 7>), dim3(grid), dim3(64 * sell_wpb()), 0, st, A.col, host_vals<T>(A), A.order, A.slice_off, A.stride, A.w_lo, s_begin, s_end, nbarg, use_order, xx, A.slice_row, A.slice_w, bb, yy, k, done, pp, zz);
-                else hipLaunchKernelGGL((k_sell<MODE, 3, T>), dim3(grid), dim3(64 * sell_wpb()), 0, st, A.col, host_vals<T>(A), A.order, A.slice_off, A.stride, A.w_lo, s_begin, s_end, nbarg, use_order, xx, A.slice_row, A.slice_w, bb, yy, k, done, pp, zz);
-                break;
-            default:
-                if (A.stride > 0 && A.w_lo == 7) hipLaunchKernelGGL((k_sell<MODE, 4, T, 7>), dim3(grid), dim3(64 * sell_wpb()), 0, st, A.col, host_vals<T>(A), A.order, A.slice_off, A.stride, A.w_lo, s_begin, s_end, nbarg, use_order, xx, A.slice_row, A.slice_w, bb, yy, k, done, pp, zz);
-                else hipLaunchKernelGGL((k_sell<MODE, 4, T>), dim3(grid), dim3(64 * sell_wpb()), 0, st, A.col, host_vals<T>(A), A.order, A.slice_off, A.stride, A.w_lo, s_begin, s_end, nbarg, use_order, xx, A.slice_row, A.slice_w, bb, yy, k, done, pp, zz);
-                break;
-        }
+        if constexpr (MODE == SELL_AX || MODE == SELL_ADD) {
+            if (A.codes) { launch_narrow<MODE, T, true>(A, kb, nb, ns, grid, nbarg, one_xcd, s_begin, s_end, use_order, xx, bb, yy, k, done, pp, zz, st); continue; }
+        }
+        launch_narrow<MODE, T, false>(A, kb, nb, ns, grid, nbarg, one_xcd, s_begin, s_end, use_order, xx, bb, yy, k, done, pp, zz, st);
     }
     if (MODE == SELL_AX && A.long_n > 0 && s_begin == 0 && s_end_in == A.n_slices && host_long_vals<T>(A)) {
-        const CoarseInit<T> zz = coarse_init<T>(zero_rows, 0, first, omega);
+        const CoarseInit<T> zz = coarse_codes<T>(A, zero_rows, 0, first, omega);
         if (k >= 8) {
             const long waves = (long)A.long_n * ((k + 63) / 64);
             hipLaunchKernelGGL((k_long_ax_cols<T>), dim3((unsigned)((waves + 3) / 4)), dim3(256), 0, st, A.long_row, A.long_ptr, A.long_col, host_long_vals<T>(A), A.long_n, x, y,
@@ -685,7 +721,7 @@
 hipError_t launch_sell_f32(SellMode mode, const SellDev& A, int s_begin, int s_end, const float* x, const float* b,
                            float* y, int k, const Ctrl* ctrl, hipStream_t st, float* zero_rows, const FirstColour* first, double omega)
 {
-    if (!A.valf || mode == SELL_RESID_SS || mode == SELL_RESID_BOTH || mode >= SELL_GS_OOP) return hipErrorInvalidValue;
+    if ((!A.valf && !A.codes) || mode == SELL_RESID_SS || mode == SELL_RESID_BOTH || mode >= SELL_GS_OOP) return hipErrorInvalidValue;
     return launch_sell_any<float>(mode, A, s_begin, s_end, x, b, y, k, ctrl, nullptr, nullptr, st, zero_rows, first, omega);
 }
 
@@ -1743,6 +1779,26 @@
     return hipGetLastError();
 }
 
+__global__ __launch_bounds__(256) void k_sell_encode(const int* __restrict__ s_col, const double* __restrict__ s_val, size_t n, double t0, double t1, double t2,
+                                                     double t3, int n_tab, int* __restrict__ out, int* bad)
+{
+    const size_t i = (size_t)blockIdx.x * 256 + threadIdx.x;
+    if (i >= n) return;
+    const int c = s_col[i];
+    if (c < 0) { out[i] = -1; return; }
+    const long long b = __double_as_longlong(s_val[i]);
+    const int code = b == __double_as_longlong(t0) ? 0 : (n_tab > 1 && b == __double_as_longlong(t1)) ? 1 : (n_tab > 2 && b == __double_as_longlong(t2)) ? 2
+                   : (n_tab > 3 && b == __double_as_longlong(t3)) ? 3 : -1;
+    if (code < 0 || c >= (1 << 29)) { atomicOr(bad, 1); out[i] = -1; return; }
+    out[i] = (c << 2) | code;
+}
+hipError_t launch_sell_encode(const SellDev& S, size_t padded, const double* tab, int n_tab, int* out_col, int* bad, hipStream_t st)
+{
+    if (padded == 0) return hipSuccess;
+    hipLaunchKernelGGL(k_sell_encode, dim3(grid1d(padded, 256)), dim3(256), 0, st, S.col, S.val, padded, tab[0], tab[1], tab[2], tab[3], n_tab, out_col, bad);
+    return hipGetLastError();
+}
+
 __global__ __launch_bounds__(256) void k_sell_diag_slots(const int* __restrict__ slice_row, const int* __restrict__ slice_off, const int* __restrict__ slice_w, int stride,
                                                          int n_slices, const int* __restrict__ s_col, int* __restrict__ slot, int* first_missing)
 {
diff --git a/surface_multigrid_code_amd/csrc/smg_device.hpp b/surface_multigrid_code_amd/csrc/smg_device.hpp
--- a/surface_multigrid_code_amd/csrc/smg_device.hpp
+++ b/surface_multigrid_code_amd/csrc/smg_device.hpp
@@ -31,6 +31,9 @@
     const int* col = nullptr;
     const double* val = nullptr;
     const float* valf = nullptr;
+    int codes = 0;
+    double tab[4] = {0.0, 0.0, 0.0, 0.0};
+    float tabf[4] = {0.0f, 0.0f, 0.0f, 0.0f};
     int long_n = 0;
     const int* long_row = nullptr;
     const int* long_ptr = nullptr;
@@ -210,6 +213,7 @@
 hipError_t launch_recipe(int n_out, const int* ptr, const int* idx, const double* coef, const double* src, double* out, hipStream_t st);
 hipError_t launch_sell_fill(const int* ptr, const int* col, const double* val, const int* perm, const int* iperm, const SellDev& S, size_t padded, hipStream_t st,
                             bool transposed = false);
+hipError_t launch_sell_encode(const SellDev& S, size_t padded, const double* tab, int n_tab, int* out_col, int* bad, hipStream_t st);
 hipError_t launch_sell_diag_slots(const SellDev& S, int* slot, int* first_missing, hipStream_t st);
 hipError_t warm_device_code(hipStream_t st);
 hipError_t launch_sell_fill_map(const int* ptr, const int* col, const int* perm, const int* iperm, const SellDev& S, size_t padded, bool transposed, int* map, hipStream_t st);
diff --git a/surface_multigrid_code_amd/csrc/smg_hier.hpp b/surface_multigrid_code_amd/csrc/smg_hier.hpp
--- a/surface_multigrid_code_amd/csrc/smg_hier.hpp
+++ b/surface_multigrid_code_amd/csrc/smg_hier.hpp
@@ -91,6 +91,7 @@
     DevBuf<double> long_val;
     DevBuf<float> long_valf;
     hipError_t upload_long(const std::vector<int>& rows, const std::vector<int>& ptr, const std::vector<int>& col, const std::vector<double>& val);
+    hipError_t encode_codes(const double* vals, size_t n_vals, hipStream_t st);
 };
 
 struct Bsr3Buf {
diff --git a/surface_multigrid_code_amd/csrc/smg_precompute.cpp b/surface_multigrid_code_amd/csrc/smg_precompute.cpp
--- a/surface_multigrid_code_amd/csrc/smg_precompute.cpp
+++ b/surface_multigrid_code_amd/csrc/smg_precompute.cpp
@@ -846,12 +846,14 @@
         const bool cut = tr_region && region && Of.color_ptr.size() > 2;
         if (!blk && Lp.P_device_filled) {
             eP = device_fill_sell(Lp.dP, Lp.P, Of.perm, Lp.ord.iperm, cut ? &Of.color_ptr : nullptr, cut, h->aux[1], h->mem_lean ? 0 : -1);
+            if (eP == hipSuccess) eP = Lp.dP.encode_codes(Lp.P.val.data(), Lp.P.val.size(), h->aux[1]);
             return;
         }
         Csr Pvi;
         if (blk) Pvi = permute(Lp.Pv, Of.perm, Lp.vord.perm);
         Sell S = build_sell(blk ? Pvi : Lp.P_int, cut ? &Of.color_ptr : nullptr, sellC, cut, h->mem_lean ? 0 : -1);
         eP = Lp.dP.upload(S);
+        if (eP == hipSuccess) eP = Lp.dP.encode_codes((blk ? Pvi : Lp.P_int).val.data(), (blk ? Pvi : Lp.P_int).val.size(), h->aux[1]);
     });
     tasks.push_back([&] {
         DeviceScope ds(h->device);
@@ -861,6 +863,7 @@
         if (!blk && Lp.PT_device_filled) {
             eQ = device_fill_sell(Lp.dPT, Lp.PT, Oc.perm, Lw.ord.iperm, cut ? &Oc.color_ptr : nullptr, cut, h->aux[2], h->mem_lean ? 0 : -1);
             if (eQ == hipSuccess) eQ = Lp.dPT.upload_long({}, {0}, {}, {});
+            if (eQ == hipSuccess) eQ = Lp.dPT.encode_codes(Lp.PT.val.data(), Lp.PT.val.size(), h->aux[2]);
             return;
         }
         Csr PTvi;
@@ -880,6 +883,7 @@
             Sell S = build_sell(M, cut ? &Oc.color_ptr : nullptr, sellC, cut, h->mem_lean ? 0 : -1);
             eQ = Lp.dPT.upload(S);
             if (eQ == hipSuccess) eQ = Lp.dPT.upload_long(lrow, lptr, lcol, lval);
+            if (eQ == hipSuccess) eQ = Lp.dPT.encode_codes(M.val.data(), M.val.size(), h->aux[2]);
             return;
         }
         Csr Ms;
```

Result: faster. 3410 V-cycles/s (median of 6 runs) (+3.1%).
